# urw7rs/diffusion-models-made-easy

Measured on AMD Instinct MI355X. Metric: denoising steps/sec + training images/sec, DDPM UNet CIFAR10 32×32 @1/2/4/8 GPU, higher is better.
Workload: dtype bf16; 1 GPU; DDPM T=1000 sampling, CIFAR10 32x32, default UNet (32,416,643 params, random init), batch 128 per GPU, t.shape=(1,); global_batch=128, parallelism=dp1 (independent chains per GPU, no data-path collective)

## Files before the change

### diffusion-models-made-easy_amd/_lib.py

```python

from __future__ import annotations

import ctypes as C
import os
import subprocess
import threading

_HERE = os.path.dirname(os.path.abspath(__file__))
LIB_PATH = os.environ.get("DMME_LIB_PATH") or os.path.join(_HERE, "libdmme_hip.so")
CSRC = os.path.join(_HERE, "csrc")

F16R32 = 4
F32, BF16, BF16X3, F16 = 0, 1, 2, 3
CHAIN_DDPM, CHAIN_DDIM, CHAIN_IDDPM, CHAIN_DDPM_GUIDED, CHAIN_DDIM_GUIDED, CHAIN_GDDIM = 0, 1, 2, 3, 4, 5
CHAIN_DDPM_CFG, CHAIN_GDDIM_CFG = 6, 7
CHAIN_DPMPP, CHAIN_DPMPP_CFG = 8, 9
CHAIN_REPAINT = 10
PRED_EPS, PRED_X0, PRED_V = 0, 1, 2
PREDICTIONS = {"eps": PRED_EPS, "x0": PRED_X0, "v": PRED_V}
THRESHOLD_NONE, THRESHOLD_STATIC, THRESHOLD_DYNAMIC = 0, 1, 2
THRESHOLDS = {"none": THRESHOLD_NONE, "static": THRESHOLD_STATIC, "dynamic": THRESHOLD_DYNAMIC}
ARCH_DDPM, ARCH_IDDPM, ARCH_CLASSIFIER, ARCH_DDPM_COND = 0, 1, 2, 3
DTYPES = {"fp32": F32, "float32": F32, "32": F32, "bf16": BF16, "bfloat16": BF16, "16": BF16, "bf16-mixed": BF16, "16-mixed": BF16,
          "bf16x3": BF16X3, "fp16": F16, "float16": F16, "half": F16, "fp16r32": F16R32}
# ... 37 lines not shown
    cmd = ["make", "-C", CSRC, "-j", str(min(8, os.cpu_count() or 1))]
    res = subprocess.run(cmd, stdout=subprocess.PIPE, stderr=subprocess.STDOUT, text=True)
    if verbose or res.returncode != 0:
        print(res.stdout)
    if res.returncode != 0:
        raise DmmeError("building libdmme_hip.so failed")
    return LIB_PATH


_vp, _i, _i64, _f, _u64 = C.c_void_p, C.c_int, C.c_int64, C.c_float, C.c_uint64

PROTOTYPES = {
    "dmme_last_error": (C.c_char_p, []),
    "dmme_version": (_i, []),
    "dmme_device_count": (_i, []),
    "dmme_unet_plan_create": (_i, [C.POINTER(UNetCfg), _i, _i, _i, _i, _i, C.POINTER(_vp)]),
    "dmme_unet_plan_destroy": (None, [_vp]),
    "dmme_unet_plan_num_params": (_i, [_vp]),
    "dmme_unet_plan_param_info": (_i, [_vp, _i, C.c_char_p, _i, C.POINTER(_i), C.POINTER(_i64), C.POINTER(_i64), C.POINTER(_i)]),
    "dmme_unet_plan_ref_numel": (_i64, [_vp]),
    "dmme_unet_plan_packed_bytes": (_i64, [_vp]),
    "dmme_unet_plan_workspace_bytes": (_i64, [_vp]),
    "dmme_unet_plan_dropmask_numel": (_i64, [_vp]),
    "dmme_unet_plan_out_channels": (_i, [_vp]),
    "dmme_unet_plan_num_launches": (_i, [_vp]),
    "dmme_unet_plan_num_launches_nograd": (_i, [_vp]),
    "dmme_unet_plan_num_folded": (_i, [_vp]),
    "dmme_unet_pack_params": (_i, [_vp, _vp, _vp, _vp]),
    "dmme_unet_pack_folded": (_i, [_vp, _vp, _vp]),
    "dmme_unet_forward": (_i, [_vp, _vp, _vp, _vp, _i, _vp, _vp, _vp, _vp]),
    "dmme_unet_forward_nograd": (_i, [_vp, _vp, _vp, _vp, _i, _vp, _vp, _vp, _vp]),
    "dmme_unet_forward_cond": (_i, [_vp, _vp, _vp, _vp, _i, _vp, _vp, _vp, _vp, _i, _vp, _vp]),
    "dmme_unet_backward_cond": (_i, [_vp, _vp, _vp, _vp, _vp, _i, _vp, _vp, _vp, _vp, _vp, _vp, _vp, _vp, _vp, _vp]),
    "dmme_unet_backward_input_cond": (_i, [_vp, _vp, _vp, _vp, _vp, _i, _vp, _vp, _vp, _vp, _vp, _vp, _vp]),
    "dmme_label_dropout": (_i, [_vp, _i, _i, _f, _u64, _u64, _vp, _vp, _vp]),
    "dmme_cfg_step": (_i, [_i, _vp, _vp, _vp, _f, _f, _f, _f, _i, _i, _i64, _vp]),
    "dmme_chain_update_cfg": (_i, [_i, _vp, _vp, _vp, _vp, _vp, _vp, _i, _i64, _vp]),
    "dmme_cfg_chain_step": (_i, [_vp, _vp, _vp, _vp, _vp, _vp, _vp, _i, _vp, _vp, _vp, _vp]),
    "dmme_dpmpp_step": (_i, [_vp, _vp, _vp, C.POINTER(_f), _i, _i, _i64, _i, _vp]),
    "dmme_chain_update_dpmpp": (_i, [_vp, _vp, _vp, _vp, _vp, _vp, _i, _i64, _i, _vp]),
    "dmme_dpmpp_chain_step": (_i, [_vp, _vp, _vp, _vp, _vp, _vp, _vp, _vp, _vp, _vp]),
    "dmme_cfg_dpmpp_step": (_i, [_vp, _vp, _vp, C.POINTER(_f), _i, _i, _i64, _vp]),
    "dmme_chain_update_cfg_dpmpp": (_i, [_vp, _vp, _vp, _vp, _vp, _vp, _i, _i64, _vp]),
    "dmme_cfg_dpmpp_chain_step": (_i, [_vp, _vp, _vp, _vp, _vp, _vp, _vp, _vp, _vp, _vp, _vp, _vp]),
    "dmme_repaint_step": (_i, [_vp, _vp, _vp, _vp, _vp, C.POINTER(_f), _i, _i64, _i, _vp]),
    "dmme_chain_update_repaint": (_i, [_vp, _vp, _vp, _vp, _vp, _vp, _vp, _vp, _i, _i64, _i, _vp]),
    "dmme_repaint_chain_step": (_i, [_vp, _vp, _vp, _vp, _vp, _vp, _vp, _vp, _vp, _vp, _vp]),
    "dmme_unet_plan_num_ops": (_i, [_vp]),
    "dmme_unet_plan_level_info": (_i, [_vp, C.c_char_p, _i]),
    "dmme_unet_plan_check": (_i, [_vp]),
    "dmme_debug_level_stamps": (_i, [_vp, _i, _i]),
    "dmme_unet_plan_op_info": (_i, [_vp, _i, C.c_char_p, _i, C.POINTER(C.c_double), C.POINTER(C.c_double)]),
    "dmme_unet_forward_profiled": (_i, [_vp, _vp, _vp, _vp, _i, _vp, _vp, _vp, _vp, _vp]),
    "dmme_unet_plan_packed_bwd_bytes": (_i64, [_vp]),
    "dmme_unet_plan_bwd_workspace_bytes": (_i64, [_vp]),
    "dmme_unet_pack_params_bwd": (_i, [_vp, _vp, _vp, _vp]),
    "dmme_unet_backward": (_i, [_vp, _vp, _vp, _vp, _vp, _i, _vp, _vp, _vp, _vp, _vp, _vp, _vp]),
    "dmme_unet_backward_buckets": (_i, [_vp, _vp, _vp, _vp, _vp, _i, _vp, _vp, _vp, _vp, _vp, _vp, _vp, BUCKET_FN, _vp]),
    "dmme_unet_backward_input": (_i, [_vp, _vp, _vp, _vp, _vp, _i, _vp, _vp, _vp, _vp, _vp, _vp]),
    "dmme_unet_plan_grad_buckets": (_i, [_vp, C.POINTER(_i64), C.POINTER(_i64), C.POINTER(_i), _i]),
    "dmme_unet_plan_bwd_summary": (_i, [_vp, C.c_char_p, _i]),
    "dmme_grad_norm": (_i, [_vp, _i64, _vp, _vp, _vp]),
    "dmme_adam_step": (_i, [_vp, _vp, _vp, _vp, _vp, _i64, _f, _f, _f, _f, _i, _vp, _f, _f, _f, _vp]),
    "dmme_amp_init": (_i, [_vp, _f, _vp]),
    "dmme_amp_scale": (_i, [_vp, _i64, _vp, _vp]),
    "dmme_adam_step_amp": (_i, [_vp, _vp, _vp, _vp, _vp, _i64, _f, _f, _f, _f, _vp, _f, _f, _f, _vp, _f, _f, _i, _vp]),
    "dmme_grad_pack_bf16": (_i, [_vp, _i64, _vp, _i64, _vp]),
    "dmme_shard_reduce_bf16": (_i, [_vp, _i, _i64, _f, _vp, _vp]),
    "dmme_grad_unpack_bf16": (_i, [_vp, _i64, _vp, _vp]),
    "dmme_unet_debug_read": (_i, [_vp, _vp, C.c_char_p, _vp, _i64, C.POINTER(_i64), _vp]),
    "dmme_unet_debug_read_grad": (_i, [_vp, _vp, C.c_char_p, _vp, _i64, C.POINTER(_i64), _vp]),
    "dmme_unet_debug_read_norm_stats": (_i, [_vp, _vp, C.c_char_p, _vp, _i64, C.POINTER(_i64), _vp]),
    "dmme_dropout_masks": (_i, [_vp, _u64, _u64, _vp, _vp]),
    "dmme_randn": (_i, [_vp, _i64, _u64, _u64, _vp]),
    "dmme_q_sample": (_i, [_vp, _vp, _vp, _vp, _vp, _i, _i64, _vp, _vp, _vp]),
    "dmme_ddpm_step": (_i, [_vp, _vp, _vp, _f, _f, _f, _i, _i64, _vp]),
    "dmme_ddim_step": (_i, [_vp, _vp, _f, _f, _i64, _vp]),
    "dmme_gddim_step": (_i, [_vp, _vp, _vp, _f, _f, _f, _i64, _vp]),
    "dmme_slerp": (_i, [_vp, _vp, _vp, _i, _i, _i64, _vp, _vp]),
    "dmme_chain_set": (_i, [_vp, _i64, _vp, _u64, _u64, _vp]),
    "dmme_chain_update": (_i, [_i, _vp, _vp, _vp, _vp, _vp, _i, _i64, _vp]),
    "dmme_chain_step": (_i, [_vp, _vp, _vp, _vp, _vp, _i, _vp, _vp, _vp, _vp]),
    "dmme_chain_update_gddim": (_i, [_vp, _vp, _vp, _vp, _vp, _vp, _i, _i64, _vp]),
    "dmme_log_softmax_grad": (_i, [_vp, _vp, _i, _i, _i, _f, _vp, _vp, _vp, _vp]),
    "dmme_chain_update_guided": (_i, [_i, _vp, _vp, _vp, _vp, _vp, _vp, _vp, _i, _i64, _vp]),
    "dmme_guided_chain_step": (_i, [_vp, _vp, _vp, _vp, _vp, _vp, _vp, _vp, _vp, _vp, _vp, _vp, _vp, _vp, _vp, _i, _vp, _vp, _vp, _vp]),
    "dmme_mse_loss": (_i, [_vp, _vp, _i64, _vp, _vp, _f, _vp, _vp]),
    "dmme_pred_to_eps": (_i, [_i, _vp, _vp, _vp, _i, _vp, _i, _i, _i64, _vp]),
    "dmme_unet_plan_set_prediction": (_i, [_vp, _i, _vp, _i]),
    "dmme_x0_threshold": (_i, [_i, _vp, _vp, _vp, _i, _vp, _i, _i, _i64, _i, _i, _f, _i, _f, _vp, _vp]),
    "dmme_x0_threshold_scratch_bytes": (_i64, [_i, _i64]),
    "dmme_x0_threshold_lds_capacity": (_i, []),
    "dmme_unet_plan_set_threshold": (_i, [_vp, _i, _vp, _i, _i, _f, _vp]),
    "dmme_q_sample_pred": (_i, [_i, _vp, _vp, _vp, _vp, _vp, _i, _i64, _vp, _vp, _vp]),
    "dmme_mse_loss_rows": (_i, [_vp, _vp, _vp, _vp, _i, _i64, _vp, _vp, _f, _vp, _vp]),
    "dmme_image_batch": (_i, [_vp, _i64, _vp, _vp, _i, _i, _i, _i, _vp, _vp]),
    "dmme_grid_tile": (_i, [_vp, _i, _i, _i, _i, _i, _i, _i, _i, _i, _i, _i, _vp, _vp]),
    "dmme_iddpm_step": (_i, [_vp, _vp, _vp, _f, _f, _f, _f, _i, _i, _i64, _vp]),
    "dmme_iddpm_loss": (_i, [_vp, _vp, _vp, _vp, _vp, _vp, _i, _i64, _f, _f, _vp, _vp, _f, _vp, _vp]),
    "dmme_iddpm_loss_rows": (_i, [_vp, _vp, _vp, _vp, _vp, _vp, _i, _vp, _i, _i64, _f, _f, _vp, _vp, _vp, _f, _vp, _vp, _vp]),
    "dmme_iddpm_prior_rows": (_i, [_vp, _i, _i64, _f, _vp, _vp]),
    "dmme_tsampler_draw": (_i, [_vp, _vp, _i, _i, _f, _u64, _u64, _i, _vp, _vp, _vp, _vp]),
    "dmme_tsampler_update": (_i, [_vp, _vp, _i, _i, _vp, _vp, _i, _vp, _vp]),
    "dmme_conv2d": (_i, [C.POINTER(ConvDesc), _vp, _vp, _vp, _vp, _vp, _vp, _vp, _vp, _vp, _vp, _i, _vp, _vp]),
    "dmme_conv2d_res": (_i, [C.POINTER(ConvDesc), _vp, _vp, _vp, _vp, _vp, _vp, _vp, _vp, _vp, _i, _i, _vp, _vp, _vp, _vp]),
    "dmme_groupnorm_scale_shift": (_i, [_i, _vp, _vp, _i, _i, _i, _i, _i, _vp, _vp, _f, _vp, _vp, _vp, _i, _vp]),
    "dmme_attention": (_i, [_i, _vp, _i, _i, _i, _vp, _i, _vp]),
    "dmme_attention_proj": (_i, [_i, _vp, _i, _i, _i, _vp, _vp, _vp, _vp, _vp, _vp, _i, _vp]),
    "dmme_attention_fold": (_i, [_i, _i, _vp, _vp, _vp, _vp, _vp, _vp, _vp, _vp, _vp]),
    "dmme_attention_block": (_i, [_i, _vp, _i, _i, _i, _vp, _i, _i, _i, _vp, _vp, _f, _vp, _vp, _vp, _vp, _vp, _vp, _vp, _vp, _vp, _i, _vp]),
    "dmme_attention_heads": (_i, [_i, _vp, _i, _i, _i, _i, _vp, _i, _vp]),
    "dmme_nchw_to_nhwc": (_i, [_i, _vp, _i, _i, _i, _vp, _vp]),
    "dmme_nhwc_to_nchw": (_i, [_i, _vp, _i, _i, _i, _vp, _vp]),
    "dmme_pack_weight": (_i, [_i, _vp, _i, _i, _i, _vp, _vp]),
    "dmme_event_create": (_i, [C.POINTER(_vp)]),
    "dmme_event_record": (_i, [_vp, _vp]),
    "dmme_event_elapsed_ms": (_i, [_vp, _vp, C.POINTER(_f)]),
    "dmme_event_destroy": (_i, [_vp]),
    "dmme_debug_set_stamps": (_i, [_vp]),
    "dmme_debug_mfma_valu": (_i, [_i, _i, _i, _vp, _vp]),
    "dmme_debug_issue_probe": (_i, [_i, _i, _i, _i, _i, _vp, _vp, _vp]),
    "dmme_debug_l2_stream": (_i, [_vp, _i64, _i, _i, _i, _i, _vp, _vp]),
}


def lib():
    global _lib
    if _lib is not None:
        return _lib
    with _lock:
        if _lib is not None:
            return _lib
        if not os.path.exists(LIB_PATH):
            raise DmmeError(
                f"{LIB_PATH} is missing: the HIP extension is not built. Run `python -c 'import __graft_entry__ as g; g.build()'` "
                "(or `make -C diffusion-models-made-easy_amd/csrc`). There is no CPU fallback for the product path."
            )
        h = C.CDLL(LIB_PATH)
        for name, (res, args) in PROTOTYPES.items():
            fn = getattr(h, name)
            fn.restype = res
            fn.argtypes = args
        _lib = h
    return _lib


def check(rc: int, what: str = ""):
    if rc != 0:
        msg = lib().dmme_last_error().decode("utf-8", "replace")
        if rc == -2:
            raise NotImplementedError(f"{what}: {msg}")
        if rc == -1:
            raise ValueError(f"{what}: {msg}")
        raise DmmeError(f"{what} failed (status {rc}): {msg}")


def require_gpu():
    if lib().dmme_device_count() <= 0:
        raise DmmeError("libdmme_hip.so loaded but no HIP device is visible; the denoiser path only runs on an MI355X")


def dtype_code(precision) -> int:
    key = str(precision).lower()
    if key not in DTYPES:
        raise ValueError(f"unknown precision {precision!r}; use 'fp32', 'bf16', 'fp16' / 'fp16r32' (inference) or 'bf16x3'")
    return DTYPES[key]
# ... 25 lines not shown
```

### diffusion-models-made-easy_amd/csrc/common.h

```cpp
#pragma once

#include <hip/hip_runtime.h>
#include <stdint.h>

#include "dmme_hip.h"

namespace dmme {

void set_error(const char* fmt, ...) __attribute__((format(printf, 1, 2)));

int debug_route(const char* key, int dflt = 0);

#define DMME_CHECK_HIP(expr)                                                                          \
    do {                                                                                              \
        hipError_t e_ = (expr);                                                                       \
        if (e_ != hipSuccess) {                                                                       \
            ::dmme::set_error("%s failed: %s (%s:%d)", #expr, hipGetErrorString(e_), __FILE__, __LINE__); \
            return DMME_ERR_HIP;                                                                      \
        }                                                                                             \
    } while (0)

#define DMME_REQUIRE(cond, code, ...)        \
    do {                                     \
        if (!(cond)) {                       \
// ... 257 lines not shown
int conv_gn_direct_query(int dtype, const ConvArgs& a, const int* cg, int n);
int launch_gn_finalize_parts(const float* part1, int tiles1, int cnt1, int C1, const float* part2, int tiles2, int cnt2, int C2, int N, int groups,
                             const float* gamma, const float* beta, float eps, float* scale, float* shift, float* mean_rstd, const float* t_shift,
                             const float* t_scale, int t_ld, int nt, hipStream_t s);

int launch_gn_generic(int dtype, const void* src1, const void* src2, int N, int HW, int C1, int C2, int groups,
                      const float* gamma, const float* beta, float eps, float* scale, float* shift, float* mean_rstd,
                      hipStream_t s);
bool gn_fast_supported(int dtype, int N, int HW, int C1, int C2, int groups);
size_t gn_fast_scratch_floats(int N, int HW, int C, int groups);
int launch_gn_fast(int dtype, const void* src1, const void* src2, int N, int HW, int C1, int C2, int groups,
                   const float* gamma, const float* beta, float eps, float* scale, float* shift, float* mean_rstd,
                   float* partial, hipStream_t s, void* act = nullptr, int act_silu = 0, const float* dmask = nullptr);
bool gn_small_act_supported(int dtype, int HW, int C1, int C2, int groups);

int launch_attn_generic(int dtype, const void* qkv, int N, int S, int C, void* out, hipStream_t s);
int launch_attn_heads(int dtype, const void* qkv, int N, int S, int C, int heads, void* out, hipStream_t s);
int launch_attn_heads_bwd(int dtype, const void* qkv, const void* dO, int N, int S, int C, int heads, float* P, float* dS, void* dqkv, hipStream_t s);
int launch_gn_modulate(float* scale, float* shift, const float* t_shift, const float* t_scale, int ld, int nt, int N, int C, hipStream_t s);
bool attn_x3_supported(int N, int S, int C, int heads);
int launch_attn_x3(const void* qkv, int N, int S, int C, int heads, void* out, hipStream_t s);
bool attn_mfma_supported(int dtype, int N, int S, int C);
bool attn_full_takes(int S, int D);
int launch_attn_mfma(int dtype, const void* qkv, int N, int S, int C, void* out, float* lse, hipStream_t s);
bool attn_proj_fusable(int dtype, int N, int S, int C, int gn_cg, int gn_tiles);
int launch_attn_proj(int dtype, const void* qkv, int N, int S, int C, void* ctx, float* lse, const void* w, const float* bias, const void* res, void* dst,
                     float* gn_part, int gn_tiles, int gn_cg, hipStream_t s, long long* stamps = nullptr);
struct AttnFoldJob {
    int64_t wq, bq, wp, bp;
    int64_t M, c, wpv, bias2;
    int32_t C, pad;
};
bool attn_fold_shape_ok(int dtype, int N, int S, int C, int gn_cg, int gn_tiles);
int launch_attn_fold(int dtype, const void* x, int N, int S, int C, const GnIn* gni, const float* scale, const float* shift, const void* M, const float* c,
                     const void* wpv, const float* bias2, const void* res, void* dst, float* gn_part, int gn_tiles, int gn_cg, hipStream_t s,
                     long long* stamps = nullptr);
int launch_attn_fold_weights(int dtype, const AttnFoldJob* jobs_dev, int n_jobs, int maxC, void* packed, hipStream_t s, const AttnFoldJob* one = nullptr);
bool attn_heads_mfma_supported(int dtype, int N, int S, int C, int heads);
int launch_attn_heads_mfma(int dtype, const void* qkv, int N, int S, int C, int heads, void* out, float* lse, hipStream_t s);
int launch_attn_heads_bwd_mfma(int dtype, const void* qkv, const void* O, const void* dO, const float* lse, int N, int S, int C, int heads, void* P,
                               void* dS, void* dqkv, hipStream_t s);
bool attn_bwd_mfma_supported(int dtype, int N, int S, int C);
int launch_attn_bwd_mfma(int dtype, const void* qkv, const void* O, const void* dO, const float* lse, int N, int S, int C, void* P, void* dS,
                         void* dqkv, hipStream_t s);

constexpr unsigned kFwdMarkKeep = 0x4B454550u, kFwdMarkNograd = 0x4E4F4752u;
constexpr unsigned kErrNogradBackward = 0x80000000u;
int launch_time_sinusoid(const int64_t* t, int nt, const float* freqs, int half, float* out, hipStream_t s, unsigned* mark = nullptr,
                         unsigned mark_val = 0);
int launch_linear_wave(int dtype, const float* in, int nt, int K, const void* W, const float* bias, int Nout,
                       int out_silu, float* out, hipStream_t s);
int launch_label_cond(const float* z2, int nt, const float* E, const int64_t* labels, int B, int K, int emb, float* temb, float* zsave, int* status,
                      hipStream_t s);
int launch_label_grad(const float* dz2, const int64_t* labels, int B, int K, int emb, float* dE, hipStream_t s);

int launch_nchw_to_nhwc(int dtype, const float* src, int N, int C, int HW, void* dst, hipStream_t s, const unsigned* mark = nullptr,
                        unsigned* err = nullptr);
int launch_nhwc_to_nchw(int dtype, const void* src, int N, int C, int HW, float* dst, hipStream_t s);
int launch_pack_weight(int dtype, const float* src, int Cout, int Cin, int taps, void* dst, hipStream_t s);
int launch_cast_f32_to_16(int dtype, const float* src, int64_t numel, void* dst, hipStream_t s);

struct PackItem {
    int64_t src_off;
    int64_t dst_off;
    int32_t cout, cin, taps;
    int32_t row0, rows;
    int32_t ci0, nci;
    int32_t as_f32;
};
int launch_pack_table(int dtype, const PackItem* items_dev, int n_items, const float* ref_flat, void* packed,
                      hipStream_t s);

int launch_randn(float* out, int64_t numel, uint64_t seed, uint64_t offset, hipStream_t s);
int launch_dropmask(float* out, int64_t numel, float p, uint64_t seed, uint64_t offset, hipStream_t s);
int launch_q_sample(const float* x0, const float* z, const float* sqrt_abar, const float* sqrt_1m_abar,
                    const int64_t* t, int B, int64_t chw, float* x_t, float* target, hipStream_t s);
int launch_pred_to_eps(int pred, float* model_out, const float* x, const float* ab, int T, const int64_t* t, int t_len, int B, int64_t chw,
                       hipStream_t s);
int launch_x0_threshold(int mode, float* out, const float* x, const float* table, int T, const int64_t* t, int t_len, int B, int64_t chw, int planes,
                        int halves, float sg, const float* sg_coef, int sg_row, int sg_col, const int64_t* sg_state, int k, float frac, void* scratch,
                        hipStream_t s);
int slerp_parts(int64_t chw);
int launch_slerp(const float* xa, const float* xb, const float* w, int n, int B, int64_t chw, float* out, float* scratch, hipStream_t s);
int launch_chain_set(void* state, int64_t i, const int64_t* t_table, uint64_t seed, uint64_t offset, hipStream_t s);

constexpr bool kind_known(int k) { return k >= DMME_CHAIN_DDPM && k <= DMME_CHAIN_REPAINT; }
constexpr bool kind_cfg(int k) { return k == DMME_CHAIN_DDPM_CFG || k == DMME_CHAIN_GDDIM_CFG || k == DMME_CHAIN_DPMPP_CFG; }
__device__ __forceinline__ float cfg_mix(float e_c, float e_u, float s) { return __fadd_rn(e_u, __fmul_rn(s, __fsub_rn(e_c, e_u))); }
constexpr int kind_base(int k) {
    return k == DMME_CHAIN_DDPM_CFG ? DMME_CHAIN_DDPM : k == DMME_CHAIN_GDDIM_CFG ? DMME_CHAIN_GDDIM : k == DMME_CHAIN_DPMPP_CFG ? DMME_CHAIN_DPMPP : k;
}
constexpr bool kind_hist(int k) { return kind_base(k) == DMME_CHAIN_DPMPP; }
constexpr bool kind_paint(int k) { return k == DMME_CHAIN_REPAINT; }
constexpr int kind_row(int k) { return kind_hist(k) || kind_paint(k) ? 8 : 4; }
constexpr int kind_scol(int k) { return kind_hist(k) ? 6 : 3; }
constexpr bool kind_grad(int k) { return k == DMME_CHAIN_DDPM_GUIDED || k == DMME_CHAIN_DDIM_GUIDED; }
constexpr int kind_planes(int k) { return k == DMME_CHAIN_IDDPM ? 2 : k == DMME_CHAIN_DPMPP || kind_paint(k) ? 0 : 1; }
enum { NOISE_NEVER, NOISE_NOT_LAST, NOISE_C2, NOISE_ROW };
constexpr int kind_noise(int k) {
    return kind_paint(k) ? NOISE_ROW : kind_hist(k) || k == DMME_CHAIN_DDIM || k == DMME_CHAIN_DDIM_GUIDED ? NOISE_NEVER : kind_base(k) == DMME_CHAIN_GDDIM ? NOISE_C2 : NOISE_NOT_LAST;
}
constexpr int kind_adds_noise(int k, float c2, int not_last) { return kind_noise(k) == NOISE_C2 ? c2 != 0.0f : kind_noise(k) == NOISE_NOT_LAST ? not_last : 0; }
constexpr int paint_streams_used(float c2, float ks, float r1) { return (c2 != 0.0f ? 1 : 0) | (ks != 0.0f ? 2 : 0) | (r1 != 0.0f ? 4 : 0); }
constexpr int kind_streams(int k) { return kind_paint(k) ? 3 : 1; }
constexpr bool kind_draws(int k, int flag, int s) { return kind_paint(k) ? ((flag >> s) & 1) != 0 : kind_noise(k) != NOISE_NEVER && flag != 0; }
constexpr bool kind_zin(int k) { return k == DMME_CHAIN_DDPM_GUIDED || kind_base(k) == DMME_CHAIN_GDDIM || k == DMME_CHAIN_DDPM_CFG || kind_paint(k); }
constexpr bool kind_ragged(int k) { return k == DMME_CHAIN_DDPM || k == DMME_CHAIN_DDIM || k == DMME_CHAIN_GDDIM || k == DMME_CHAIN_IDDPM; }

struct SamplerOperands {
    float* x;
    const float* out;
    const float* grad;
    const float* zin;
    float* hist;
    const float* known;
    const float* mask;
    int64_t chw, numel, n4;
    int planes;
};
int launch_sampler_eager(const char* what, int kind, const SamplerOperands& o, const float* row, int flag, hipStream_t s);
int launch_sampler_chain(const char* what, int kind, const SamplerOperands& o, const float* coef, const int64_t* t_table, void* state, hipStream_t s);
int launch_label_dropout(const int64_t* labels, int B, int K, float p, uint64_t seed, uint64_t offset, int64_t* out, int* status, hipStream_t s);
int launch_cls_head_fwd(int dtype, const void* top, int B, int HW, int C, int G, const float* gamma, const float* beta, const float* W,
                        const float* bias, int K, float* logits, hipStream_t s);
int launch_cls_head_bwd(int dtype, const void* top, int B, int HW, int C, int G, const float* gamma, const float* beta, const float* W, int K,
                        const float* dlog, void* dtop, float* pooled, float* rows, hipStream_t s);
int launch_cls_head_wgrad(const float* dlog, const float* pooled, const float* rows, int B, int K, int C, float* dW, float* db, float* dgamma,
                          float* dbeta, hipStream_t s);
int launch_log_softmax_grad(const float* logits, const int64_t* y, int B, int K, int mode, float scale, float* loss, float* dlog, int* status,
                            hipStream_t s);
int launch_image_batch(const uint8_t* data, const int64_t* idx, const uint8_t* flip, int B, int C, int H, int W, float* out, hipStream_t s);
int launch_grid_tile(const float* x, int B, int C, int H, int W, int cell0, int cell_stride, int xmaps, int ymaps, int pad, int out_kind, int raw,
                     void* canvas, hipStream_t s);
int launch_iddpm_loss(const float* out, const float* x_t, const float* x_0, const float* target, const int64_t* t, const float* coef, int B,
                      int64_t chw, float w_simple, float w_vlb, float* loss, float* d_out, float gscale, float* scratch, hipStream_t s);
int launch_iddpm_loss_rows(const float* out, const float* x_t, const float* x_0, const float* target, const int64_t* t, const float* coef, int T,
                           const float* weight, int B, int64_t chw, float w_simple, float w_vlb, float* loss, float* rows, float* d_out,
                           float gscale, int* status, float* scratch, hipStream_t s);
int launch_iddpm_prior_rows(const float* x_0, int B, int64_t chw, float alpha_bar_T, float* prior, hipStream_t s);
int launch_tsampler_draw(const float* hist, const int* count, int T, int H, float uniform_prob, uint64_t seed, uint64_t offset, int B, int64_t* t,
                         float* weight, float* p, hipStream_t s);
int launch_tsampler_update(float* hist, int* count, int T, int H, const int64_t* t, const float* L, int B, int* status, hipStream_t s);
int launch_mse(const float* eps, const float* target, int64_t numel, float* loss, float* d_eps, float gscale,
               float* scratch, hipStream_t s);

int launch_wgrad_generic(int dtype, const ConvArgs& a, const void* dY, float* dW, hipStream_t s);
bool wgrad_small_supported(int dtype, const ConvArgs& a);
int launch_wgrad_small(int dtype, const ConvArgs& a, const void* dY, float* dW, hipStream_t s);
bool wgrad_mfma_supported(int dtype, const ConvArgs& a);
int launch_wgrad_mfma(int dtype, const ConvArgs& a, const void* dY, float* dWp, hipStream_t s);
struct PackItem;

struct WgLayer {
    int64_t src1_off, src2_off;
    int64_t scale_off, shift_off;
    int64_t dmask_off;
    int64_t dy_off;
    int64_t dw_off;
    int64_t act_off;
    int act_bws;
    int N, Hin, Win, C1, C2, up, Hout, Wout, Cout, pro_silu;
    int shTW, shTH;
    int ks_off[4], half_off;
    int ks_row[4], half_row;
    ConvTile g;
};
struct WgJob {
    int layer, cot, cit, tile0, ntiles;
};
bool wgrad_group_layer(int dtype, const ConvArgs& a, WgLayer& L, int* co_tile, int* ci_tile);
int launch_wgrad_group(int dtype, int taps, const WgLayer* layers_dev, const WgJob* jobs_dev, int njobs, const void* ws, const void* bws,
                       const float* drop_masks, float* wimage, hipStream_t s, int dma = 0, const void* zero_page = nullptr);
int launch_wgrad_unpack(const PackItem* items_dev, int n_items, const float* image, float* grad_flat, hipStream_t s);
int launch_colsum(int dtype, const void* dY, int N, int HW, int C, float* rowsum, float* dbias, float* dtproj, int ld, int nt,
                  hipStream_t s);
struct GnMod {
    const float* t_scale = nullptr;
    const float* beta = nullptr;
    float* d_shift = nullptr;
    float* d_scale = nullptr;
    int ld = 0, nt = 0;
#if defined(__HIPCC__)
    __device__ __forceinline__ float mul(int n, int c) const { return t_scale ? 1.0f + t_scale[(int64_t)(nt == 1 ? 0 : n) * ld + c] : 1.0f; }
    __device__ __forceinline__ void emit(int n, int c, float A, float B, float gamma_c) const {
        if (!t_scale) return;
        const float ds = fmaf(gamma_c, B, beta[c] * A);
        if (nt == 1) {
            atomicAdd(&d_shift[c], A);
            atomicAdd(&d_scale[c], ds);
        } else {
            d_shift[(int64_t)n * ld + c] = A;
            d_scale[(int64_t)n * ld + c] = ds;
        }
    }
#endif
};
int launch_gn_bwd_generic(int dtype, const void* dv, const void* x1, const void* x2, int N, int HW, int C1, int C2, int groups,
                          const float* gamma, const float* mean_rstd, const float* scale, const float* shift, const float* dmask,
                          int pro_silu, void* dx1, void* dx2, int acc1, int acc2, float* dgamma, float* dbeta, GnMod mod, hipStream_t s);
bool colsum_fast_supported(int dtype, int HW, int C);
struct BiasJob {
    int64_t rowsum_off;
    int64_t dbias_off;
    int C, cblock, tcol;
// ... 56 lines not shown
```

### diffusion-models-made-easy_amd/csrc/kernels_sampler.hip

```cpp
#include "common.h"

#include <type_traits>

namespace dmme {

struct Philox {
    uint32_t c[4];
    uint32_t k[2];
};
__device__ __forceinline__ void philox_round(uint32_t (&c)[4], uint32_t k0, uint32_t k1) {
    const uint64_t p0 = (uint64_t)0xD2511F53u * c[0];
    const uint64_t p1 = (uint64_t)0xCD9E8D57u * c[2];
    const uint32_t n0 = (uint32_t)(p1 >> 32) ^ c[1] ^ k0;
    const uint32_t n1 = (uint32_t)p1;
    const uint32_t n2 = (uint32_t)(p0 >> 32) ^ c[3] ^ k1;
    const uint32_t n3 = (uint32_t)p0;
    c[0] = n0;
    c[1] = n1;
    c[2] = n2;
    c[3] = n3;
}
__device__ __forceinline__ void philox4x32_10(uint64_t seed, uint64_t ctr, uint32_t (&out)[4]) {
    uint32_t c[4] = {(uint32_t)ctr, (uint32_t)(ctr >> 32), 0u, 0u};
    uint32_t k0 = (uint32_t)seed, k1 = (uint32_t)(seed >> 32);
// ... 61 lines not shown
    if (numel <= 0) return DMME_OK;
    hipLaunchKernelGGL(dropmask_kernel, dim3(grid_for((numel + 3) / 4)), dim3(256), 0, s, out, numel, p, seed, offset);
    DMME_CHECK_LAUNCH();
    return DMME_OK;
}

__global__ void __launch_bounds__(256) q_sample_kernel(const float* __restrict__ x0, const float* __restrict__ z,
                                                       const float* __restrict__ sqrt_abar,
                                                       const float* __restrict__ sqrt_1m_abar,
                                                       const int64_t* __restrict__ t, int64_t chw, int64_t total,
                                                       float* __restrict__ x_t, float* __restrict__ target) {
    for (int64_t i = blockIdx.x * (int64_t)blockDim.x + threadIdx.x; i < total; i += (int64_t)gridDim.x * blockDim.x) {
        const int64_t tn = t[i / chw];
        const float sa = sqrt_abar[tn], sd = sqrt_1m_abar[tn];
        const float mean = sa * x0[i];
        const float xt = mean + sd * z[i];
        x_t[i] = xt;
        if (target) target[i] = (xt - mean) / sd;
    }
}
int launch_q_sample(const float* x0, const float* z, const float* sqrt_abar, const float* sqrt_1m_abar,
                    const int64_t* t, int B, int64_t chw, float* x_t, float* target, hipStream_t s) {
    const int64_t total = (int64_t)B * chw;
    if (total <= 0) return DMME_OK;
    hipLaunchKernelGGL(q_sample_kernel, dim3(grid_for(total)), dim3(256), 0, s, x0, z, sqrt_abar, sqrt_1m_abar, t, chw, total,
                       x_t, target);
    DMME_CHECK_LAUNCH();
    return DMME_OK;
}

__device__ __forceinline__ float ddpm_mean(float x, float e, float c0, float c1) { return __fmul_rn(c0, __fsub_rn(x, __fmul_rn(c1, e))); }
__device__ __forceinline__ float ddim_collapse(float x, float e, float c0, float c1) {
    return __fmul_rn(c1, __fdiv_rn(__fsub_rn(x, __fmul_rn(c0, e)), c1));
}
__device__ __forceinline__ float iddpm_std(float v, float log_beta, float log_beta_tilde) {
    return sqrtf(expf(__fadd_rn(__fmul_rn(v, log_beta), __fmul_rn(__fsub_rn(1.0f, v), log_beta_tilde))));
}
template <int KIND>
__device__ __forceinline__ float sampler_update(float x, float e, float v, float g, float z, float c0, float c1, float c2, float c3, int add_noise) {
    if (KIND == DMME_CHAIN_DDIM) return ddim_collapse(x, e, c0, c1);
    if (KIND == DMME_CHAIN_DDIM_GUIDED) return ddim_collapse(x, __fsub_rn(e, __fmul_rn(c2, g)), c0, c1);
    float m;
    if (KIND == DMME_CHAIN_GDDIM) {
        m = __fadd_rn(__fmul_rn(c0, x), __fmul_rn(c1, e));
    } else {
        m = ddpm_mean(x, e, c0, c1);
        if (KIND == DMME_CHAIN_DDPM_GUIDED) m = __fadd_rn(m, __fmul_rn(c3, g));
    }
    return add_noise ? __fadd_rn(m, __fmul_rn(KIND == DMME_CHAIN_IDDPM ? iddpm_std(v, c2, c3) : c2, z)) : m;
}
struct DpmppRow {
    float q0, q1, k0, k1, w, clip, s;
};
__device__ __forceinline__ float dpmpp_update(float x, float e, float prev, const DpmppRow& r, bool valid, float& x0) {
    x0 = __fadd_rn(__fmul_rn(r.q0, x), __fmul_rn(r.q1, e));
    if (r.clip != 0.0f) x0 = fminf(fmaxf(x0, -1.0f), 1.0f);
    const float d = valid ? __fadd_rn(x0, __fmul_rn(r.w, __fsub_rn(x0, prev))) : x0;
    return __fadd_rn(__fmul_rn(r.k0, x), __fmul_rn(r.k1, d));
}
struct PaintRow {
    float c0, c1, c2, ka, ks, r0, r1;
};
__device__ __forceinline__ float paint_update(float x, float e, float x0, float m, float z0, float z1, float z2, const PaintRow& r, int used) {
    float u = ddpm_mean(x, e, r.c0, r.c1);
    if (used & 1) u = __fadd_rn(u, __fmul_rn(r.c2, z0));
    float k = __fmul_rn(r.ka, x0);
    if (used & 2) k = __fadd_rn(k, __fmul_rn(r.ks, z1));
    const float y = __fadd_rn(__fmul_rn(m, k), __fmul_rn(__fsub_rn(1.0f, m), u));
    return used & 4 ? __fadd_rn(__fmul_rn(r.r0, y), __fmul_rn(r.r1, z2)) : y;
}
__device__ __forceinline__ float4 load4(const float* p) { return *reinterpret_cast<const float4*>(p); }

struct ChainState {
    long long i;
    long long t;
    unsigned long long offset;
    unsigned long long seed;
    unsigned int ticket, pad;
    unsigned long long history_valid;
    unsigned long long reserved[2];
};
static_assert(sizeof(ChainState) == 64, "ChainState is eight 64-bit words (dmme_hip.h: dmme_chain_*)");

__global__ void chain_set_kernel(ChainState* st, long long i, const long long* __restrict__ t_table, unsigned long long seed, unsigned long long offset) {
    st->i = i;
    st->t = t_table[i];
    st->offset = offset;
    st->seed = seed;
    st->ticket = 0u;
    st->pad = 0u;
    st->history_valid = 0ull;
}
int launch_chain_set(void* state, int64_t i, const int64_t* t_table, uint64_t seed, uint64_t offset, hipStream_t s) {
    hipLaunchKernelGGL(chain_set_kernel, dim3(1), dim3(1), 0, s, (ChainState*)state, (long long)i, (const long long*)t_table, (unsigned long long)seed,
                       (unsigned long long)offset);
    DMME_CHECK_LAUNCH();
    return DMME_OK;
}

__device__ __forceinline__ void chain_advance(ChainState* st, const long long* __restrict__ t_table, long long i, unsigned long long offset_inc,
                                              bool raise_history) {
    if (threadIdx.x != 0) return;
    const unsigned tk = atomicAdd(&st->ticket, 1u);
    if (tk != gridDim.x - 1) return;
    const long long ni = i > 0 ? i - 1 : 0;
    st->i = ni;
    st->t = t_table[ni];
    if (offset_inc) st->offset += offset_inc;
    if (raise_history) st->history_valid = 1ull;
    atomicExch(&st->ticket, 0u);
}

struct Row {
    float c[8];
};

template <bool DRAWS>
__device__ __forceinline__ void noise4(bool add_noise, const float* zin, int64_t b, uint64_t seed, uint64_t ctr, float (&z)[4]) {
    z[0] = z[1] = z[2] = z[3] = 0.f;
    if (!add_noise) return;
    if (!DRAWS || zin) {
        const float4 zv = load4(zin + b);
        z[0] = zv.x; z[1] = zv.y; z[2] = zv.z; z[3] = zv.w;
    } else {
        normal4(seed, ctr, z);
    }
}

template <int KIND, bool DRAWS>
__device__ __forceinline__ void step_noise(const SamplerOperands& o, int flag, const float* zin, int64_t q, uint64_t seed, uint64_t off,
                                           float (&z)[4 * kind_streams(KIND)]) {
    if constexpr (kind_streams(KIND) == 1) {
        noise4<DRAWS>(kind_draws(KIND, flag, 0), zin, q * 4, seed, off + (uint64_t)q, z);
    } else {
#pragma unroll
        for (int s = 0; s < kind_streams(KIND); ++s)
            noise4<DRAWS>(kind_draws(KIND, flag, s), zin ? zin + s * o.numel : nullptr, q * 4, seed, off + (uint64_t)s * (uint64_t)o.n4 + (uint64_t)q,
                          *reinterpret_cast<float(*)[4]>(z + 4 * s));
    }
}

template <int KIND>
__device__ __forceinline__ void update_quad(const SamplerOperands& o, int64_t q, const Row& r, int flag, const float (&z)[4 * kind_streams(KIND)]) {
    const int64_t b = q * 4;
    const int planes = kind_planes(KIND) ? kind_planes(KIND) : o.planes;
    const int64_t eo = planes == 2 ? b + (b / o.chw) * o.chw : b;
    float4 xv = load4(o.x + b), ev = load4(o.out + eo), av = make_float4(0.f, 0.f, 0.f, 0.f);
    float *xs = reinterpret_cast<float*>(&xv), *es = reinterpret_cast<float*>(&ev), *as = reinterpret_cast<float*>(&av);
    if constexpr (kind_cfg(KIND)) {
        const float4 uv = load4(o.out + o.n4 * 4 + b);
        const float* us = reinterpret_cast<const float*>(&uv);
#pragma unroll
        for (int j = 0; j < 4; ++j) es[j] = cfg_mix(es[j], us[j], r.c[kind_scol(KIND)]);
    }
    if constexpr (kind_hist(KIND)) {
        const DpmppRow d = {r.c[0], r.c[1], r.c[2], r.c[3], r.c[4], r.c[5], r.c[6]};
        if (flag) av = load4(o.hist + b);
#pragma unroll
        for (int j = 0; j < 4; ++j) xs[j] = dpmpp_update(xs[j], es[j], as[j], d, flag != 0, as[j]);
        *reinterpret_cast<float4*>(o.hist + b) = av;
    } else if constexpr (kind_paint(KIND)) {
        const PaintRow p = {r.c[0], r.c[1], r.c[2], r.c[3], r.c[4], r.c[5], r.c[6]};
        const float4 mv = load4(o.mask + b);
        av = load4(o.known + b);
        const float* ms = reinterpret_cast<const float*>(&mv);
#pragma unroll
        for (int j = 0; j < 4; ++j) xs[j] = paint_update(xs[j], es[j], as[j], ms[j], z[j], z[4 + j], z[8 + j], p, flag);
    } else {
        constexpr bool LEARNED = KIND == DMME_CHAIN_IDDPM;
        if (LEARNED && flag) av = load4(o.out + eo + o.chw);
        if (kind_grad(KIND)) av = load4(o.grad + b);
#pragma unroll
        for (int j = 0; j < 4; ++j)
            xs[j] = sampler_update<kind_base(KIND)>(xs[j], es[j], LEARNED ? as[j] : 0.f, kind_grad(KIND) ? as[j] : 0.f, z[j], r.c[0], r.c[1], r.c[2],
                                                    kind_cfg(KIND) ? 0.f : r.c[3], flag);
    }
    *reinterpret_cast<float4*>(o.x + b) = xv;
    if (kind_cfg(KIND)) *reinterpret_cast<float4*>(o.x + o.n4 * 4 + b) = xv;
}

template <int KIND>
__global__ void __launch_bounds__(256) eager_kernel(SamplerOperands o, Row r, int flag) {
    const bool quads_fit = KIND != DMME_CHAIN_IDDPM || o.chw % 4 == 0;
    for (int64_t q = blockIdx.x * (int64_t)blockDim.x + threadIdx.x; q < o.n4; q += (int64_t)gridDim.x * blockDim.x) {
        const int64_t b = q * 4;
        if (!kind_ragged(KIND) || (b + 3 < o.numel && quads_fit)) {
            float z[4 * kind_streams(KIND)];
            step_noise<KIND, false>(o, flag, o.zin, q, 0, 0, z);
            update_quad<KIND>(o, q, r, flag, z);
        } else if constexpr (kind_ragged(KIND)) {
            for (int64_t i = b; i < b + 4 && i < o.numel; ++i) {
                const int64_t eo = KIND == DMME_CHAIN_IDDPM ? i + (i / o.chw) * o.chw : i;
                o.x[i] = sampler_update<KIND>(o.x[i], o.out[eo], KIND == DMME_CHAIN_IDDPM && flag ? o.out[eo + o.chw] : 0.f, 0.f, flag ? o.zin[i] : 0.f,
                                              r.c[0], r.c[1], r.c[2], r.c[3], flag);
            }
        }
    }
}

template <int KIND>
__global__ void __launch_bounds__(256) __attribute__((amdgpu_waves_per_eu(8))) chain_kernel(SamplerOperands o, const float* __restrict__ coef, const long long* __restrict__ t_table, ChainState* st) {
    const long long i = st->i, t = st->t;
    const unsigned long long off = st->offset, seed = st->seed;
    Row r;
#pragma unroll
    for (int j = 0; j < kind_row(KIND); ++j) r.c[j] = coef[kind_row(KIND) * i + j];
    const int flag = kind_hist(KIND) ? st->history_valid != 0ull : kind_paint(KIND) ? paint_streams_used(r.c[2], r.c[4], r.c[6]) : kind_adds_noise(KIND, r.c[2], t != 1);
    for (int64_t q = blockIdx.x * (int64_t)blockDim.x + threadIdx.x; q < o.n4; q += (int64_t)gridDim.x * blockDim.x) {
        float z[4 * kind_streams(KIND)];
        step_noise<KIND, true>(o, flag, kind_zin(KIND) ? o.zin : nullptr, q, seed, off, z);
        update_quad<KIND>(o, q, r, flag, z);
    }
    __syncthreads();
    chain_advance(st, t_table, i, kind_hist(KIND) ? 0ull : (unsigned long long)o.n4 * kind_streams(KIND), kind_hist(KIND));
}

template <int K = 0, class F>
static int dispatch_kind(int kind, F&& f) {
    if constexpr (K > DMME_CHAIN_REPAINT) {
        set_error("unknown sampler kind %d", kind);
        return DMME_ERR_INVALID;
    } else {
        return kind == K ? f(std::integral_constant<int, K>{}) : dispatch_kind<K + 1>(kind, f);
    }
}
static int check_operands(const char* what, int kind, const SamplerOperands& o, bool eager) {
    DMME_REQUIRE(kind_known(kind), DMME_ERR_INVALID, "%s: unknown sampler kind %d", what, kind);
    DMME_REQUIRE(o.x && o.out && (o.hist || !kind_hist(kind)) && ((o.known && o.mask) || !kind_paint(kind)) && o.numel > 0 && o.chw > 0, DMME_ERR_INVALID,
                 "%s: bad argument", what);
    DMME_REQUIRE(kind_grad(kind) == (o.grad != nullptr), DMME_ERR_INVALID, "%s: the guided kinds (3, 4) and only they take a gradient", what);
    DMME_REQUIRE(kind_planes(kind) || o.planes == 1 || o.planes == 2, DMME_ERR_INVALID, "%s: a network output of %d planes per image (1: eps, 2: eps and v)",
                 what, o.planes);
    DMME_REQUIRE((eager && kind_ragged(kind)) || o.chw % 4 == 0, DMME_ERR_UNSUPPORTED, "%s: image size %lld is not a multiple of 4", what, (long long)o.chw);
    return DMME_OK;
}
int launch_sampler_eager(const char* what, int kind, const SamplerOperands& o, const float* row, int flag, hipStream_t s) {
    if (kind_ragged(kind) && o.numel <= 0) return DMME_OK;
    if (int rc = check_operands(what, kind, o, true)) return rc;
    DMME_REQUIRE(row, DMME_ERR_INVALID, "%s: null argument", what);
    Row r = {};
    for (int j = 0; j < kind_row(kind); ++j) r.c[j] = row[j];
    if (!kind_hist(kind)) flag = kind_paint(kind) ? paint_streams_used(r.c[2], r.c[4], r.c[6]) : kind_adds_noise(kind, r.c[2], flag);
    DMME_REQUIRE(o.zin || kind_hist(kind) || !flag, DMME_ERR_INVALID, "%s: a step that adds noise needs z", what);
    return dispatch_kind(kind, [&](auto k) -> int {
        constexpr int K = decltype(k)::value;
        if constexpr (kind_grad(K)) {
            set_error("%s: the guided kinds have no eager form", what);
            return DMME_ERR_INVALID;
        } else {
            hipLaunchKernelGGL(eager_kernel<K>, dim3(grid_for(o.n4)), dim3(256), 0, s, o, r, flag);
            DMME_CHECK_LAUNCH();
            return DMME_OK;
        }
    });
}
int launch_sampler_chain(const char* what, int kind, const SamplerOperands& o, const float* coef, const int64_t* t_table, void* state, hipStream_t s) {
    if (int rc = check_operands(what, kind, o, false)) return rc;
    DMME_REQUIRE(coef && t_table && state, DMME_ERR_INVALID, "%s: null argument", what);
    return dispatch_kind(kind, [&](auto k) -> int {
        hipLaunchKernelGGL(chain_kernel<decltype(k)::value>, dim3(grid_for(o.n4)), dim3(256), 0, s, o, coef, (const long long*)t_table, (ChainState*)state);
        DMME_CHECK_LAUNCH();
        return DMME_OK;
    });
}

__global__ void __launch_bounds__(256) mse_partial_kernel(const float* __restrict__ eps, const float* __restrict__ target,
                                                          int64_t numel, float* __restrict__ d_eps, float gscale,
                                                          float* __restrict__ partial) {
    __shared__ float red[16];
    float acc = 0.f;
    for (int64_t i = blockIdx.x * (int64_t)blockDim.x + threadIdx.x; i < numel; i += (int64_t)gridDim.x * blockDim.x) {
        const float d = target[i] - eps[i];
        acc += d * d;
        if (d_eps) d_eps[i] = (-2.0f * d) * gscale;
    }
    const float tot = block_sum(acc, red);
    if (threadIdx.x == 0) partial[blockIdx.x] = tot;
}
__global__ void __launch_bounds__(256) mse_final_kernel(const float* partial, int n, float inv_numel, float* loss) {
    __shared__ float red[16];
    float acc = 0.f;
    for (int i = threadIdx.x; i < n; i += blockDim.x) acc += partial[i];
    const float tot = block_sum(acc, red);
    if (threadIdx.x == 0) loss[0] = tot * inv_numel;
}
int launch_mse(const float* eps, const float* target, int64_t numel, float* loss, float* d_eps, float gscale,
               float* scratch, hipStream_t s) {
    DMME_REQUIRE(numel > 0, DMME_ERR_INVALID, "mse: numel must be positive");
    unsigned g = grid_for(numel);
    if (g > 1024) g = 1024;
    hipLaunchKernelGGL(mse_partial_kernel, dim3(g), dim3(256), 0, s, eps, target, numel, d_eps,
                       gscale / (float)numel, scratch);
    DMME_CHECK_LAUNCH();
    hipLaunchKernelGGL(mse_final_kernel, dim3(1), dim3(256), 0, s, scratch, (int)g, 1.0f / (float)numel, loss);
    DMME_CHECK_LAUNCH();
    return DMME_OK;
}

__device__ __forceinline__ void iddpm_loss_elem(const float* __restrict__ c, bool t_is_one, float e, float v, float xt, float x0, float tgt,
                                                float& d, float& vlb, float& dv) {
    d = tgt - e;
    const float mean = c[0] * (xt - c[1] * e);
    const float sd = iddpm_std(v, c[2], c[3]);
    const float hl = 0.5f * (c[2] - c[3]);
    if (t_is_one) {
        const float ap = (x0 + 1.0f / 255.0f - mean) / sd, am = (x0 - 1.0f / 255.0f - mean) / sd;
        const bool up = x0 < 1.0f, lo = x0 > -1.0f;
        const float Fp = up ? 0.5f * (1.0f + erff(ap * 0.70710678118654752f)) : 1.0f;
        const float Fm = lo ? 0.5f * (1.0f + erff(am * 0.70710678118654752f)) : 0.0f;
        const float prob = Fp - Fm;
        vlb = -logf(fmaxf(prob, 1e-12f));
        const float pp = up ? 0.3989422804014327f * expf(-0.5f * ap * ap) * ap : 0.f;
        const float pm = lo ? 0.3989422804014327f * expf(-0.5f * am * am) * am : 0.f;
        dv = prob >= 1e-12f ? hl * (pp - pm) / prob : 0.f;
    } else {
        const float qm = c[4] * x0 + c[5] * xt;
        const float q = c[6] / sd, ratio = q * q;
        const float u = (qm - mean) / sd, t1 = u * u;
        vlb = 0.5f * (ratio + t1 - 1.0f - logf(ratio));
        dv = hl * (1.0f - ratio - t1);
    }
}
__global__ void __launch_bounds__(256) iddpm_loss_kernel(const float* __restrict__ out, const float* __restrict__ x_t, const float* __restrict__ x_0,
                                                         const float* __restrict__ target, const int64_t* __restrict__ t,
                                                         const float* __restrict__ coef, int64_t chw, int64_t total, float w_simple, float w_vlb,
                                                         float gscale, float* __restrict__ d_out, float* __restrict__ partial) {
    __shared__ float red[16];
    float acc_s = 0.f, acc_v = 0.f;
    for (int64_t i = blockIdx.x * (int64_t)blockDim.x + threadIdx.x; i < total; i += (int64_t)gridDim.x * blockDim.x) {
        const int64_t b = i / chw, r = i - b * chw;
        const int64_t tt = t[b];
        float d, vlb, dv;
        iddpm_loss_elem(coef + tt * 8, tt == 1, out[b * 2 * chw + r], out[b * 2 * chw + chw + r], x_t[i], x_0[i], target[i], d, vlb, dv);
        acc_s += d * d;
        acc_v += vlb;
        if (d_out) {
            d_out[b * 2 * chw + r] = (-2.0f * d) * (w_simple * gscale);
            d_out[b * 2 * chw + chw + r] = dv * (w_vlb * gscale);
        }
    }
    const float ts = block_sum(acc_s, red);
    __syncthreads();
    const float tv = block_sum(acc_v, red);
// ... 471 lines not shown
```

### diffusion-models-made-easy_amd/csrc/plan.h

```cpp
#pragma once
#include <stdarg.h>
#include <stdlib.h>
#include <stdio.h>
#include <string.h>

#include <algorithm>
#include <memory>
#include <string>
#include <unordered_map>
#include <vector>

#include "common.h"
#include "lvl.h"

namespace dmme {

static inline int64_t align_up(int64_t v, int64_t a) { return (v + a - 1) / a * a; }

template <typename T>
class DevTable {
    T* p_ = nullptr;

public:
    DevTable() = default;
// ... 115 lines not shown
    DevTable<unsigned> sync_dev;
    double flops = 0, bytes = 0;
};

}

using namespace dmme;

struct dmme_plan {
    dmme_unet_cfg cfg;
    int B, H, W, dtype, device;
    int x3 = 0;
    int mix = 0;
    int out_channels = 0;
    int head_src = -1, p_hgw = -1, p_hgb = -1, p_hw = -1, p_hb = -1;
    int64_t bws_hpool = 0, bws_hrows = 0;
    int cond = 0, p_lemb = -1, label_op = -1;
    std::vector<Param> params;
    std::vector<Tensor> tensors;
    std::vector<Op> ops;
    std::unordered_map<std::string, int> named;
    int64_t ref_numel = 0, packed_bytes = 0, ws_bytes = 0, dropmask_numel = 0;
    int64_t ws_tsin = 0, ws_th1 = 0, ws_temb = 0, ws_tproj = 0, ws_gnpart = 0;
    int64_t ws_mark = 0;
    int64_t ws_tz1 = -1, ws_tz2 = -1;
    int64_t ws_splitk = 0, splitk_floats = 0;
    int tproj_cols = 0;
    int64_t tproj_w_off = 0, tproj_b_off = 0;
    int freqs_param = -1;
    DevTable<PackItem> items_dev;
    int n_items = 0;
    int n_launches = 0;
    struct TBlock { int tw, tb, col, cout; };
    std::vector<TBlock> tblocks;
    int p_l1w = -1, p_l1b = -1, p_l2w = -1, p_l2b = -1;
    int64_t packed_bwd_bytes = 0, bws_bytes = 0;
    std::vector<int64_t> gt_off;
    int64_t bws_zero = 0, bws_zero_bytes = 0, bws_wimage = 0, bws_gnS = 0, bws_zpage = 0;
    DevTable<PackItem> items_unpack_dev;
    int n_items_unpack = 0;
    int64_t bws_sink = 0, sink_half = 0;
    int64_t bws_tmp = 0, bws_dy = 0, bws_rowsum = 0, bws_dtproj = 0, bws_dtemb = 0, bws_dh1 = 0, bws_z = 0, bws_wT = 0, bws_attP = 0,
            bws_attdS = 0;
    DevTable<PackItem> items_bwd_dev;
    int n_items_bwd = 0;
    struct WgGroup {
        int taps = 0;
        std::vector<WgLayer> layers;
        std::vector<WgJob> jobs;
        DevTable<WgLayer> layers_dev;
        DevTable<WgJob> jobs_dev;
        int dma = 0;
        int stride = 1;
    } wg[3];
    struct GradBucket {
        int op_lo = 0, op_hi = 0;
        WgGroup wg[3];
        int col0 = 0, col1 = 0, bias0 = 0, bias1 = 0;
        std::vector<std::pair<int, int>> unpack, tcols;
        std::vector<std::pair<int64_t, int64_t>> ranges;
    };
    std::vector<GradBucket> gb;
    std::vector<int64_t> tp_tiles;
    DevTable<int64_t> tp_tiles_dev;
    int tp_n64 = 0;
    std::vector<BiasJob> bias_jobs;
    DevTable<BiasJob> bias_jobs_dev;
    std::vector<ColJob> col_jobs;
    DevTable<ColJob> col_jobs_dev;
    std::vector<LvlRun> lvl_runs;
    int lvl_max_wg = LVL_MAX_WG;
    PinnedWord err_host;
    mutable const void* nograd_ws = nullptr;
    std::vector<AttnFoldJob> fold_jobs;
    DevTable<AttnFoldJob> fold_jobs_dev;
    int fold_maxC = 0, n_launches_nograd = 0;
    mutable const void* fold_packed = nullptr;
    int pred = DMME_PRED_EPS, pred_T = 0;
    const float* pred_ab = nullptr;
    int thr_mode = DMME_THRESHOLD_NONE, thr_T = 0, thr_k = 0;
    float thr_frac = 0.f;
    const float* thr_table = nullptr;
    void* thr_scratch = nullptr;
};

namespace dmme {

constexpr int kR32TwoPassDefault = 0;
static inline int conv_dt(const dmme_plan* P, const Op& o) { return o.route_f32 ? DMME_F32 : P->dtype; }
static inline int wg_index(const Op& o) { return o.taps == 1 ? 1 : o.stride == 2 ? 2 : 0; }

void fill_conv(const dmme_plan* P, const Op& o, const char* packed, const float* x, float* y, char* ws, const float* drop_masks, int nt, ConvArgs& a,
               bool fwd = false);
bool gn_from_parts(const dmme_plan* P, const Op& o);
void assign_levels(dmme_plan* P);
void assign_rseg(dmme_plan* P);
int run_level(const dmme_plan* P, const LvlRun& R, const char* pk, char* ws, int nt, const float* drop_masks, hipStream_t s, bool keep_ctx = true);
void assign_lvl_nograd(dmme_plan* P);
void assign_attn_fold(dmme_plan* P);
int lvl_check(const dmme_plan* P, const char* where, hipStream_t stream = nullptr, bool have_stream = false);
void build_unpack_items(const dmme_plan* P, std::vector<PackItem>& items);
void plan_backward(dmme_plan* P);

}
```

### diffusion-models-made-easy_amd/csrc/plan.hip

```cpp
#include "plan.h"

#include <functional>
#include <map>
#include <mutex>

namespace dmme {

static thread_local char g_err[512] = "";
void set_error(const char* fmt, ...) {
    va_list ap;
    va_start(ap, fmt);
    vsnprintf(g_err, sizeof(g_err), fmt, ap);
    va_end(ap);
}

int debug_route(const char* key, int dflt) {
    const char* e = getenv("DMME_DEBUG_ROUTE");
    if (!e || !*e) return dflt;
    const size_t kl = strlen(key);
    for (const char* p = e; *p;) {
        const char* end = strchr(p, ',');
        const size_t len = end ? (size_t)(end - p) : strlen(p);
        if (len >= kl && !strncmp(p, key, kl) && (len == kl || p[kl] == '=')) return len == kl ? 1 : atoi(p + kl + 1);
        if (!end) break;
// ... 470 lines not shown
            const int64_t v = (int64_t)B * to.H * to.W * (cin > to.C ? cin : to.C);
            if (v > mx) mx = v;
        }
        P->splitk_floats = 4 * mx;
        P->ws_splitk = ws_alloc(P->splitk_floats * 4 + 16);
    }
    P->ws_bytes = ws;
    P->n_launches = (int)ops.size();

    return DMME_OK;
}

static void push_pack_items(const Param& p, int64_t dst_off, int as_f32, bool wide_co, std::vector<PackItem>& items) {
    const int LIMIT = 8192;
    int nco, nci;
    if (as_f32 == 1) {
        nci = p.cin;
        nco = LIMIT / (p.cin * p.taps);
        if (nco < 1) nco = 1;
    } else if (wide_co) {
        nco = p.cout < 64 ? p.cout : 64;
        nci = LIMIT / (nco * p.taps);
        if (nci > p.cin) nci = p.cin;
        if (nci >= 4) nci &= ~3;
        if (nci < 1) nci = 1;
    } else {
        nci = p.cin;
        if (nci * p.taps > LIMIT) nci = LIMIT / p.taps;
        nco = LIMIT / (nci * p.taps);
        if (nco < 1) nco = 1;
    }
    if (as_f32 != 1 && nco > 256) nco = 256;
    for (int r0 = 0; r0 < p.cout; r0 += nco)
        for (int c0 = 0; c0 < p.cin; c0 += nci) {
            PackItem it;
            it.src_off = p.ref_off;
            it.dst_off = dst_off;
            it.cout = p.cout;
            it.cin = p.cin;
            it.taps = p.taps;
            it.row0 = r0;
            it.rows = p.cout - r0 < nco ? p.cout - r0 : nco;
            it.ci0 = c0;
            it.nci = p.cin - c0 < nci ? p.cin - c0 : nci;
            it.as_f32 = as_f32;
            items.push_back(it);
        }
}

void build_pack_items(const dmme_plan* P, std::vector<PackItem>& items) {
    for (const Param& p : P->params) push_pack_items(p, p.packed_off, p.pack_code >= 0 ? p.pack_code : p.as_f32 ? 1 : 0, false, items);
}

void build_pack_items_bwd(const dmme_plan* P, std::vector<PackItem>& items) {
    for (const Param& p : P->params)
        if (p.packed_bwd_off >= 0) push_pack_items(p, p.packed_bwd_off, 2, true, items);
}

void build_unpack_items(const dmme_plan* P, std::vector<PackItem>& items) {
    const int64_t CHUNK = 16384;
    for (const Param& p : P->params) {
        if (p.wp_off < 0) continue;
        const int64_t row = (int64_t)p.cin * p.taps;
        int64_t rows_per = CHUNK / row;
        if (rows_per < 1) rows_per = 1;
        for (int64_t r0 = 0; r0 < p.cout; r0 += rows_per) {
            PackItem it;
            it.src_off = p.ref_off;
            it.dst_off = p.wp_off;
            it.cout = p.cout;
            it.cin = p.cin;
            it.taps = p.taps;
            it.row0 = (int32_t)r0;
            it.rows = (int32_t)((p.cout - r0) < rows_per ? (p.cout - r0) : rows_per);
            it.ci0 = 0;
            it.nci = p.cin;
            it.as_f32 = 0;
            items.push_back(it);
        }
    }
}

void fill_conv(const dmme_plan* P, const Op& o, const char* packed, const float* x, float* y, char* ws,
               const float* drop_masks, int nt, ConvArgs& a, bool fwd) {
    const int64_t es = (int64_t)dtype_size(P->dtype);
    (void)es;
    a.x3 = P->x3 || o.route_f32;
    a.f16 = P->dtype == DMME_F16 && !o.route_f32;
    a.mix = o.mix;
    a.mix2 = o.mix2;
    a.N = P->B;
    if (o.src1 == -2) {
        a.src1 = x;
        a.in_nchw = 1;
        a.C1 = P->cfg.in_channels;
        a.Hin = P->H;
        a.Win = P->W;
    } else {
        const Tensor& t = P->tensors[o.src1];
        a.src1 = ws + t.off;
        a.C1 = t.C;
        a.Hin = t.H;
        a.Win = t.W;
    }
    if (o.src2 >= 0) {
        a.src2 = ws + P->tensors[o.src2].off;
        a.C2 = P->tensors[o.src2].C;
    }
    const Param& w = P->params[o.w];
    a.w = packed + w.packed_off;
    a.bias = (const float*)(packed + P->params[o.b].packed_off);
    a.Cout = w.cout;
    a.taps = o.taps;
    a.stride = o.stride;
    a.up = o.up;
    const int Hv = o.up ? 2 * a.Hin : a.Hin, Wv = o.up ? 2 * a.Win : a.Win;
    a.Hout = Hv / o.stride;
    a.Wout = Wv / o.stride;
    if (o.gn >= 0) {
        a.scale = (const float*)(ws + P->ops[o.gn].gn_scale);
        a.shift = (const float*)(ws + P->ops[o.gn].gn_shift);
        const Op& g = P->ops[o.gn];
        if (fwd && g.gn_in_consumer) {
            const Tensor& t1 = P->tensors[g.gn_src1];
            const Tensor* t2 = g.gn_src2 >= 0 ? &P->tensors[g.gn_src2] : nullptr;
            a.has_gni = 1;
            a.gni.p1 = (const float*)(ws + t1.stats_off);
            a.gni.t1 = t1.stats_tiles;
            a.gni.cnt1 = t1.stats_cnt;
            a.gni.C1 = t1.C;
            a.gni.p2 = t2 ? (const float*)(ws + t2->stats_off) : nullptr;
            a.gni.t2 = t2 ? t2->stats_tiles : 0;
            a.gni.cnt2 = t2 ? t2->stats_cnt : 0;
            a.gni.C2 = t2 ? t2->C : 0;
            a.gni.groups = P->cfg.num_groups;
            a.gni.gamma = (const float*)(packed + P->params[g.gn_gamma].packed_off);
            a.gni.beta = (const float*)(packed + P->params[g.gn_beta].packed_off);
            a.gni.eps = 1e-5f;
            a.gni.mean_rstd = (float*)(ws + g.gn_mr);
            if (g.gn_mod_col >= 0) {
                a.gni.t_shift = (const float*)(ws + P->ws_tproj) + g.gn_mod_col;
                a.gni.t_scale = a.gni.t_shift + g.gn_mod_C;
                a.gni.t_ld = P->tproj_cols;
                a.gni.nt = nt;
            }
        }
    }
    a.pro_silu = o.pro_silu;
    a.out_silu = o.out_silu;
    if (o.dmask_off >= 0 && drop_masks) a.dmask = drop_masks + o.dmask_off;
    if (fwd && o.use_act) {
        a.src1 = ws + P->ops[o.gn].gn_act;
        a.C1 = a.C1 + a.C2;
        a.src2 = nullptr;
        a.C2 = 0;
        a.scale = a.shift = a.dmask = nullptr;
        a.pro_silu = 0;
    }
    if (o.tproj_col >= 0) {
        a.tproj = (const float*)(ws + P->ws_tproj) + o.tproj_col;
        a.tproj_ld = P->tproj_cols;
        a.nt = nt;
    }
    if (fwd && o.rseg >= 0) {
        const Op& rc = P->ops[o.rseg];
        const Tensor& r1 = P->tensors[rc.src1];
        a.r_src1 = ws + r1.off;
        a.r_C1 = r1.C;
        if (rc.src2 >= 0) {
            a.r_src2 = ws + P->tensors[rc.src2].off;
            a.r_C2 = P->tensors[rc.src2].C;
        }
        a.r_w = packed + P->params[rc.w].packed_off;
        a.r_bias = (const float*)(packed + P->params[rc.b].packed_off);
    } else if (o.res1 >= 0) {
        a.res1 = ws + P->tensors[o.res1].off;
        a.R1 = P->tensors[o.res1].C;
        if (o.res2 >= 0) a.res2 = ws + P->tensors[o.res2].off;
    }
    if (P->splitk_floats > 0 && ws) {
        a.splitk = (float*)(ws + P->ws_splitk);
        a.splitk_cap = P->splitk_floats;
    }
    if (fwd && o.gd_n > 0) {
        a.n_gno = o.gd_n;
        a.gn_eps = 1e-5f;
        a.gn_cg = P->tensors[o.dst].C / P->cfg.num_groups;
        for (int k = 0; k < o.gd_n; ++k) {
            const Op& g = P->ops[o.gd_gn[k]];
            GnOut& G = a.gno[k];
            G.gamma = (const float*)(packed + P->params[g.gn_gamma].packed_off);
            G.beta = (const float*)(packed + P->params[g.gn_beta].packed_off);
            G.scale = (float*)(ws + g.gn_scale);
            G.shift = (float*)(ws + g.gn_shift);
            G.mean_rstd = (float*)(ws + g.gn_mr);
            G.C = P->tensors[g.gn_src1].C + (g.gn_src2 >= 0 ? P->tensors[g.gn_src2].C : 0);
            G.cg = G.C / P->cfg.num_groups;
            G.c_off = o.gd_coff[k];
            if (k == o.gd_act) {
                const Op& cv = P->ops[g.gn_consumer];
                a.act = ws + g.gn_act;
                a.act_k = k;
                a.act_silu = cv.pro_silu;
                a.act_dmask = (cv.dmask_off >= 0 && drop_masks) ? drop_masks + cv.dmask_off : nullptr;
            }
        }
    }
    a.gn_raw_moments = P->mix ? 1 : 0;
    if (o.dst == -2) {
        a.dst = y;
        a.out_nchw = 1;
    } else {
        const Tensor& td = P->tensors[o.dst];
        a.dst = ws + td.off;
        if (td.stats_off >= 0) {
            a.gn_part = (float*)(ws + td.stats_off);
            a.gn_cg = td.C / P->cfg.num_groups;
            a.gn_tiles = td.stats_tiles;
        }
    }
}

bool gn_from_parts(const dmme_plan* P, const Op& o) {
    if (o.gn_force_small) return false;
    const Tensor& t1 = P->tensors[o.gn_src1];
    if (t1.stats_off < 0) return false;
    const int G = P->cfg.num_groups;
    int C = t1.C;
    if (o.gn_src2 >= 0) {
        const Tensor& t2 = P->tensors[o.gn_src2];
        if (t2.stats_off < 0) return false;
        C += t2.C;
        const int cg = C / G;
        if (t1.C % cg || cg % (t1.C / G) || cg % (t2.C / G)) return false;
    }
    return true;
}

void assign_stats(dmme_plan* P) {
    std::vector<char> wanted(P->tensors.size(), 0);
    for (const Op& o : P->ops)
        if (o.kind == OP_GN && o.lvl < 0) {
            wanted[o.gn_src1] = 1;
// ... 178 lines not shown
            rc.fused_away = 1;
        }
    next:;
    }
}

void assign_attn_proj(dmme_plan* P) {
    if (P->x3) return;
    for (int ai = 0; ai + 1 < (int)P->ops.size(); ++ai) {
        Op& at = P->ops[ai];
        if (at.kind != OP_ATTN || at.lvl >= 0 || at.at_heads != 1) continue;
        Op& pr = P->ops[ai + 1];
        if (pr.kind != OP_CONV || pr.src1 != at.at_out || pr.src2 >= 0 || pr.taps != 1 || pr.lvl >= 0 || pr.gn >= 0 || pr.pro_silu || pr.out_silu || pr.dmask_off >= 0 ||
            pr.tproj_col >= 0 || pr.res1 < 0 || pr.res2 >= 0 || pr.up || pr.stride != 1 || pr.gd_n > 0 || pr.mix || pr.route_f32 || pr.dst < 0 || pr.fused_away || pr.rseg >= 0)
            continue;
        const Tensor &q = P->tensors[at.at_qkv], &td = P->tensors[pr.dst];
        if (q.f32 || td.f32 || P->tensors[pr.res1].f32 || P->tensors[at.at_out].f32) continue;
        const int S = q.H * q.W, C = q.C / 3;
        if (td.C != C || P->tensors[pr.res1].C != C) continue;
        const bool stats = td.stats_off >= 0;
        if (!attn_proj_fusable(P->dtype, P->B, S, C, stats ? td.C / P->cfg.num_groups : 0, stats ? td.stats_tiles : 0)) continue;
        at.at_proj = ai + 1;
        pr.fused_away = 2;
    }
}

void assign_attn_fold(dmme_plan* P) {
    if (getenv("DMME_NO_ATTN_FOLD") || debug_route("no_attn_fold") || !is16(P->dtype) || P->x3 || P->mix) return;
    int64_t cur = P->packed_bytes;
    const int64_t es = (int64_t)dtype_size(P->dtype);
    for (int ai = 1; ai < (int)P->ops.size(); ++ai) {
        Op& at = P->ops[ai];
        if (at.kind != OP_ATTN || at.at_proj < 0 || at.at_heads != 1 || at.lvl >= 0) continue;
        Op& qc = P->ops[ai - 1];
        const Op& pr = P->ops[at.at_proj];
        if (qc.kind != OP_CONV || qc.dst != at.at_qkv || qc.taps != 1 || qc.src1 < 0 || qc.src2 >= 0 || qc.gn < 0 || qc.pro_silu || qc.out_silu || qc.dmask_off >= 0 ||
            qc.tproj_col >= 0 || qc.res1 >= 0 || qc.res2 >= 0 || qc.up || qc.stride != 1 || qc.gd_n > 0 || qc.mix || qc.route_f32 || qc.fused_away || qc.rseg >= 0 ||
            qc.use_act || qc.lvl >= 0 || pr.res1 != qc.src1)
            continue;
        const Op& gn = P->ops[qc.gn];
        const Tensor& tx = P->tensors[qc.src1];
        const int C = tx.C, groups = P->cfg.num_groups;
        if (gn.kind != OP_GN || gn.gn_src1 != qc.src1 || gn.gn_src2 >= 0 || gn.gn_mod_col >= 0 || gn.gn_act >= 0 || tx.f32 ||
            (gn.gn_in_consumer && (tx.stats_off < 0 || tx.stats_tiles > 32)) || P->tensors[at.at_qkv].C != 3 * C || P->params[qc.w].pack_code >= 0 || P->params[pr.w].pack_code >= 0)
            continue;
        bool only_here = true;
        for (int oi = 0; oi < (int)P->ops.size() && only_here; ++oi) {
            const Op& o = P->ops[oi];
            if (oi == ai) continue;
            if (o.kind == OP_CONV && (o.src1 == at.at_qkv || o.src2 == at.at_qkv || o.res1 == at.at_qkv || o.res2 == at.at_qkv)) only_here = false;
            if (o.kind == OP_GN && (o.gn_src1 == at.at_qkv || o.gn_src2 == at.at_qkv)) only_here = false;
            if (o.kind == OP_ATTN && o.at_qkv == at.at_qkv) only_here = false;
            if (o.kind == OP_CAST && o.cast_src == at.at_qkv) only_here = false;
        }
        const Tensor& td = P->tensors[pr.dst];
        const bool stats = td.stats_off >= 0;
        if (!only_here || !attn_fold_shape_ok(P->dtype, P->B, tx.H * tx.W, C, stats ? C / groups : 0, stats ? td.stats_tiles : 0)) continue;
        at.at_fold_qkv = ai - 1;
        qc.folded_into = ai;
        at.fold_M = cur;
        cur = align_up(cur + (int64_t)C * C * es, 256);
        at.fold_wpv = cur;
        cur = align_up(cur + (int64_t)C * C * es, 256);
        at.fold_c = cur;
        cur = align_up(cur + (int64_t)C * 4, 256);
        at.fold_b2 = cur;
        cur = align_up(cur + (int64_t)C * 4, 256);
        AttnFoldJob jb{};
        jb.wq = P->params[qc.w].packed_off;
        jb.bq = P->params[qc.b].packed_off;
        jb.wp = P->params[pr.w].packed_off;
        jb.bp = P->params[pr.b].packed_off;
        jb.M = at.fold_M;
        jb.c = at.fold_c;
        jb.wpv = at.fold_wpv;
        jb.bias2 = at.fold_b2;
        jb.C = C;
        P->fold_jobs.push_back(jb);
        if (C > P->fold_maxC) P->fold_maxC = C;
    }
    P->packed_bytes = cur;
}

int run_gn(const dmme_plan* P, const Op& o, const char* pk, char* ws, int nt, const float* drop_masks, hipStream_t s) {
    if (o.gn_direct || o.gn_in_consumer) return DMME_OK;
    const float* tsh = o.gn_mod_col >= 0 ? (const float*)(ws + P->ws_tproj) + o.gn_mod_col : nullptr;
    const float* tsc = tsh ? tsh + o.gn_mod_C : nullptr;
    int rc;
    const Tensor& t1 = P->tensors[o.gn_src1];
    const void* s1 = ws + t1.off;
    const void* s2 = o.gn_src2 >= 0 ? ws + P->tensors[o.gn_src2].off : nullptr;
    const int C2 = o.gn_src2 >= 0 ? P->tensors[o.gn_src2].C : 0;
    const float* gam = (const float*)(pk + P->params[o.gn_gamma].packed_off);
    const float* bet = (const float*)(pk + P->params[o.gn_beta].packed_off);
    float* sc = (float*)(ws + o.gn_scale);
    float* sh = (float*)(ws + o.gn_shift);
    if (gn_from_parts(P, o)) {
        const Tensor* t2 = o.gn_src2 >= 0 ? &P->tensors[o.gn_src2] : nullptr;
        return launch_gn_finalize_parts((const float*)(ws + t1.stats_off), t1.stats_tiles, t1.stats_cnt, t1.C,
                                        t2 ? (const float*)(ws + t2->stats_off) : nullptr, t2 ? t2->stats_tiles : 0,
                                        t2 ? t2->stats_cnt : 0, C2, P->B, P->cfg.num_groups, gam, bet, 1e-5f, sc, sh,
                                        (float*)(ws + o.gn_mr), tsh, tsc, P->tproj_cols, nt, s);
    }
    const int gdt = t1.f32 ? DMME_F32 : P->dtype;
    if (gn_fast_supported(gdt, P->B, t1.H * t1.W, t1.C, C2, P->cfg.num_groups)) {
        void* act = nullptr;
        int act_silu = 0;
        const float* dm = nullptr;
        if (o.gn_act >= 0) {
            const Op& cv = P->ops[o.gn_consumer];
            act = ws + o.gn_act;
            act_silu = cv.pro_silu;
            if (cv.dmask_off >= 0 && drop_masks) dm = drop_masks + cv.dmask_off;
        }
        rc = launch_gn_fast(gdt, s1, s2, P->B, t1.H * t1.W, t1.C, C2, P->cfg.num_groups, gam, bet, 1e-5f, sc, sh,
                            (float*)(ws + o.gn_mr), (float*)(ws + P->ws_gnpart), s, act, act_silu, dm);
    }
    else
        rc = launch_gn_generic(gdt, s1, s2, P->B, t1.H * t1.W, t1.C, C2, P->cfg.num_groups, gam, bet, 1e-5f, sc, sh,
                               (float*)(ws + o.gn_mr), s);
    if (rc != DMME_OK || !tsh) return rc;
    return launch_gn_modulate(sc, sh, tsh, tsc, P->tproj_cols, nt, P->B, o.gn_mod_C, s);
}

int run_op(const dmme_plan* P, const Op& o, const char* pk, const float* x, const int64_t* t, int nt, float* y,
           char* ws, const float* drop_masks, hipStream_t s, bool keep_ctx, const int64_t* labels = nullptr, int* status = nullptr) {
    if (o.lvl >= 0) return o.lvl_first ? run_level(P, P->lvl_runs[o.lvl], pk, ws, nt, drop_masks, s, keep_ctx) : DMME_OK;
    if (o.fused_away) return DMME_OK;
    const bool fold = !keep_ctx && P->fold_packed == (const void*)pk;
    if (fold && o.kind == OP_CONV && o.folded_into >= 0) return DMME_OK;
    switch (o.kind) {
        case OP_SINUS:
            return launch_time_sinusoid(t, nt, (const float*)(pk + P->params[P->freqs_param].packed_off),
                                        P->cfg.pos_dim / 2, (float*)(ws + P->ws_tsin), s, (unsigned*)(ws + P->ws_mark),
                                        keep_ctx ? kFwdMarkKeep : kFwdMarkNograd);
        case OP_LINEAR: {
            const char* w = o.lin_w >= 0 ? pk + P->params[o.lin_w].packed_off : pk + P->tproj_w_off;
            const float* b = (const float*)(o.lin_b >= 0 ? pk + P->params[o.lin_b].packed_off : pk + P->tproj_b_off);
            if (nt > 4)
                return launch_small_gemm(P->dtype, 0, (const float*)(ws + o.lin_in), o.lin_K, w, o.lin_K, nt, o.lin_N, o.lin_K, b, o.lin_silu,
                                         (float*)(ws + o.lin_out), o.lin_N, s, o.lin_pre >= 0 ? (float*)(ws + o.lin_pre) : nullptr);
            return launch_linear_wave(P->dtype, (const float*)(ws + o.lin_in), nt, o.lin_K, w, b, o.lin_N, o.lin_silu,
                                      (float*)(ws + o.lin_out), s);
        }
        case OP_LABEL: {
            float* z2 = (float*)(ws + P->ws_tz2);
            return launch_label_cond(z2, nt, (const float*)(pk + P->params[P->p_lemb].packed_off), labels, P->B, P->cfg.num_classes, P->cfg.emb_dim,
                                     (float*)(ws + P->ws_temb), nt == P->B ? z2 : nullptr, status, s);
        }
        case OP_GN:
            return run_gn(P, o, pk, ws, nt, drop_masks, s);
        case OP_CONV: {
            ConvArgs a{};
            fill_conv(P, o, pk, x, y, ws, drop_masks, nt, a, true);
            return launch_conv(conv_dt(P, o), a, s);
        }
        case OP_CAST: {
            const Tensor& ts = P->tensors[o.cast_src];
            return launch_cast_f32_to_16(P->dtype, (const float*)(ws + ts.off), (int64_t)P->B * ts.H * ts.W * ts.C, ws + P->tensors[o.cast_dst].off, s);
        }
        case OP_ATTN: {
            const Tensor& q = P->tensors[o.at_qkv];
            const int S = q.H * q.W, C = q.C / 3;
            if (fold && o.at_fold_qkv >= 0) {
                ConvArgs a{}, qa{};
                fill_conv(P, P->ops[o.at_proj], pk, x, y, ws, drop_masks, nt, a, true);
                fill_conv(P, P->ops[o.at_fold_qkv], pk, x, y, ws, drop_masks, nt, qa, true);
                return launch_attn_fold(P->dtype, qa.src1, P->B, S, C, qa.has_gni ? &qa.gni : nullptr, qa.scale, qa.shift, pk + o.fold_M, (const float*)(pk + o.fold_c), pk + o.fold_wpv,
                                        (const float*)(pk + o.fold_b2), a.res1, a.dst, a.gn_part, a.gn_tiles, a.gn_cg, s);
            }
            if (o.at_proj >= 0) {
                ConvArgs a{};
                fill_conv(P, P->ops[o.at_proj], pk, x, y, ws, drop_masks, nt, a, true);
                return launch_attn_proj(P->dtype, ws + q.off, P->B, S, C, keep_ctx ? ws + P->tensors[o.at_out].off : nullptr, (float*)(ws + o.at_lse), a.w, a.bias,
                                        a.res1, a.dst, a.gn_part, a.gn_tiles, a.gn_cg, s);
            }
            if (P->x3 && attn_x3_supported(P->B, S, C, o.at_heads))
                return launch_attn_x3(ws + q.off, P->B, S, C, o.at_heads, ws + P->tensors[o.at_out].off, s);
            if (o.at_heads > 1) {
                if (attn_heads_mfma_supported(P->dtype, P->B, S, C, o.at_heads))
                    return launch_attn_heads_mfma(P->dtype, ws + q.off, P->B, S, C, o.at_heads, ws + P->tensors[o.at_out].off, (float*)(ws + o.at_lse), s);
                return launch_attn_heads(P->dtype, ws + q.off, P->B, S, C, o.at_heads, ws + P->tensors[o.at_out].off, s);
            }
            if (attn_mfma_supported(P->dtype, P->B, S, C))
                return launch_attn_mfma(P->dtype, ws + q.off, P->B, S, C, ws + P->tensors[o.at_out].off, (float*)(ws + o.at_lse), s);
            return launch_attn_generic(P->dtype, ws + q.off, P->B, S, C, ws + P->tensors[o.at_out].off, s);
        }
    }
    return DMME_OK;
}
void op_account(const dmme_plan* P, const Op& o, char* label, int cap, double* flops, double* bytes) {
    const double es = (double)dtype_size(P->dtype);
    const char* tn = P->dtype == DMME_BF16 ? "bf16" : P->dtype == DMME_F16 ? "f16" : "float";
    const double B = P->B;
    *flops = 0;
    *bytes = 0;
    if (o.lvl >= 0) {
        const LvlRun& R = P->lvl_runs[o.lvl];
        if (o.lvl_first) {
            snprintf(label, cap, "lvl_engine_kernel<%dx%d>", 1 << R.sh, 1 << R.sh);
            *flops = R.flops;
            *bytes = R.bytes;
        } else {
            snprintf(label, cap, "(level engine)");
        }
        return;
    }
    if (o.fused_away) {
        snprintf(label, cap, o.fused_away == 2 ? "(proj 1x1 conv inside its block's attention launch)" : "(residual 1x1 conv inside its block's conv2)");
        return;
    }
    switch (o.kind) {
        case OP_SINUS:
            snprintf(label, cap, "time_sinusoid_kernel");
            break;
        case OP_LABEL:
            snprintf(label, cap, "label_cond_kernel");
            *flops = B * P->cfg.emb_dim;
            *bytes = 4.0 * B * P->cfg.emb_dim * 3;
            break;
        case OP_LINEAR:
            snprintf(label, cap, "linear_wave_kernel<%s>", tn);
            *flops = 2.0 * o.lin_K * o.lin_N;
            *bytes = (double)o.lin_K * o.lin_N * es + 4.0 * (o.lin_K + 2.0 * o.lin_N);
            break;
        case OP_GN: {
            const Tensor& t1 = P->tensors[o.gn_src1];
            const int C = t1.C + (o.gn_src2 >= 0 ? P->tensors[o.gn_src2].C : 0);
            const bool fast = gn_fast_supported(P->dtype, P->B, t1.H * t1.W, t1.C, C - t1.C, P->cfg.num_groups);
            if (o.gn_direct || o.gn_in_consumer) {
                snprintf(label, cap, o.gn_direct ? "(norm finished by its producers' epilogues)" : "(norm finished by its consumer's parameter fill)");
            } else if (gn_from_parts(P, o)) {
                snprintf(label, cap, "gn_finalize_parts_kernel");
                *bytes = 2.0 * B * C * 4;
            } else {
                snprintf(label, cap, fast ? "gn_partial_kernel<%s>" : "gn_generic_kernel<%s>", tn);
                *bytes = B * t1.H * t1.W * C * es + 2.0 * B * C * 4;
            }
            break;
        }
        case OP_CONV: {
            ConvArgs a{};
            fill_conv(P, o, (const char*)4096, (const float*)4096, (float*)4096, (char*)4096, nullptr, 1, a, true);
            const int cdt = conv_dt(P, o);
            conv_label(conv_route(cdt, a), cdt, a, label, cap);
            const double Cin = a.C1 + a.C2, opix = B * a.Hout * a.Wout;
            *flops = 2.0 * opix * a.Cout * Cin * a.taps;
            *bytes = B * a.Hin * a.Win * Cin * (a.in_nchw ? 4.0 : es) + opix * a.Cout * (a.out_nchw ? 4.0 : es) +
                     (double)a.Cout * Cin * a.taps * es + (a.res1 ? opix * a.Cout * es : 0.0);
            if (a.r_w) {
                const double Cres = a.r_C1 + a.r_C2;
                *flops += 2.0 * opix * a.Cout * Cres;
                *bytes += opix * Cres * es + (double)a.Cout * Cres * es;
            }
            break;
        }
// ... 46 lines not shown
        DMME_REQUIRE(cfg->num_classes >= 1, DMME_ERR_INVALID, "plan_create: classifier num_classes=%d", cfg->num_classes);
        DMME_REQUIRE(cfg->channels_per_depth[cfg->num_depths - 1] <= 1024, DMME_ERR_UNSUPPORTED, "plan_create: classifier head wider than 1024 channels");
    }
    if (cfg->arch == DMME_ARCH_IDDPM) {
        DMME_REQUIRE(cfg->num_heads >= 1, DMME_ERR_INVALID, "plan_create: num_heads must be >= 1");
    }
    for (int d = 0; d < cfg->num_depths; ++d)
        DMME_REQUIRE(cfg->channels_per_depth[d] > 0 && cfg->channels_per_depth[d] % cfg->num_groups == 0,
                     DMME_ERR_INVALID, "channels_per_depth[%d]=%d not divisible by num_groups=%d", d,
                     cfg->channels_per_depth[d], cfg->num_groups);
    return DMME_OK;
}

static int check_mix_kernels(const dmme_plan* P) {
    if (!P->mix) return DMME_OK;
    for (const Op& o : P->ops) {
        if (o.kind != OP_CONV || !(o.mix || o.route_f32)) continue;
        ConvArgs a{};
        fill_conv(P, o, (const char*)4096, (const float*)4096, (float*)4096, (char*)4096, nullptr, 1, a);
        const bool ok = !o.mix || conv_route(P->dtype, a).family == (o.mix == 3 ? CONV_THIN : o.mix == 4 ? CONV1X1_SPLIT : CONV3X3_SPLIT);
        DMME_REQUIRE(ok, DMME_ERR_UNSUPPORTED, "plan_create: precision fp16r32 has no kernel for the %dx%d conv %d+%d -> %d channels on the %dx%d level (B = %d)",
                     o.taps == 9 ? 3 : 1, o.taps == 9 ? 3 : 1, a.C1, a.C2, a.Cout, a.Hout, a.Wout, P->B);
    }
    return DMME_OK;
}

static int count_launches(const dmme_plan* P, bool nograd = false) {
    int n = 0;
    for (const Op& o : P->ops) {
        if (o.fused_away || (nograd && o.folded_into >= 0)) continue;
        if (o.lvl >= 0)
            n += o.lvl_first;
        else if (o.kind == OP_GN)
            n += !(o.gn_direct || o.gn_in_consumer);
        else
            ++n;
    }
    return n;
}

#define DMME_TRY(expr)                 \
    do {                               \
        if (int rc_ = (expr)) return rc_; \
    } while (0)

static int upload_tables(dmme_plan* P) {
    DMME_CHECK_HIP(hipSetDevice(P->device));
    std::vector<PackItem> items, bitems, uitems;
    build_pack_items(P, items);
    build_pack_items_bwd(P, bitems);
    build_unpack_items(P, uitems);
    P->n_items = (int)items.size();
    P->n_items_bwd = (int)bitems.size();
    P->n_items_unpack = (int)uitems.size();
    DMME_TRY(P->items_dev.upload(items));
    DMME_TRY(P->items_bwd_dev.upload(bitems));
    DMME_TRY(P->items_unpack_dev.upload(uitems));
    DMME_TRY(P->tp_tiles_dev.upload(P->tp_tiles));
    DMME_TRY(P->col_jobs_dev.upload(P->col_jobs));
    DMME_TRY(P->bias_jobs_dev.upload(P->bias_jobs));
    if (!P->fold_jobs.empty()) DMME_TRY(P->fold_jobs_dev.upload(P->fold_jobs));
    std::vector<dmme_plan::WgGroup*> all_groups{&P->wg[0], &P->wg[1], &P->wg[2]};
    for (auto& B_ : P->gb)
        for (int k = 0; k < 3; ++k) all_groups.push_back(&B_.wg[k]);
    for (dmme_plan::WgGroup* G : all_groups) {
        if (G->jobs.empty()) continue;
        DMME_TRY(G->layers_dev.upload(G->layers));
        DMME_TRY(G->jobs_dev.upload(G->jobs));
    }
    DMME_TRY(P->err_host.alloc());
    for (LvlRun& R : P->lvl_runs) {
        DMME_TRY(R.ops_dev.upload(R.ops));
        if (R.raw_skipped > 0) DMME_TRY(R.ops_nograd_dev.upload(R.ops_nograd));
        DMME_TRY(R.sync_dev.zeroed(16 + R.ops.size() * 2 * (size_t)R.NG * LVL_NS));
    }
    return DMME_OK;
}

}

extern "C" {

DMME_API const char* dmme_last_error(void) { return g_err; }
DMME_API int dmme_version(void) { return 115; }
DMME_API int dmme_device_count(void) {
    int n = 0;
    if (hipGetDeviceCount(&n) != hipSuccess) return 0;
    return n;
}

DMME_API int dmme_unet_plan_create(const dmme_unet_cfg* cfg, int B, int H, int W, int dtype, int device, dmme_plan** out) {
    DMME_REQUIRE(cfg && out, DMME_ERR_INVALID, "plan_create: null argument");
    DMME_TRY(check_cfg(cfg, B, H, W, dtype));
    std::unique_ptr<dmme_plan> owned(new dmme_plan());
    dmme_plan* P = owned.get();
    P->cfg = *cfg;
    if (cfg->arch == DMME_ARCH_DDPM_COND) {
        P->cond = 1;
        P->cfg.arch = DMME_ARCH_DDPM;
    }
    P->B = B;
    P->H = H;
    P->W = W;
    P->x3 = dtype == DMME_BF16X3;
    P->mix = dtype == DMME_F16R32;
    P->dtype = P->x3 ? DMME_F32 : P->mix ? DMME_F16 : dtype;
    P->device = device;
    DMME_TRY(build_plan(P));
    DMME_TRY(check_mix_kernels(P));
    assign_levels(P);
    const bool fused_gn = !getenv("DMME_NO_FUSED_GN");
    if (fused_gn) assign_stats(P);
    if (fused_gn && !getenv("DMME_NO_GN_DIRECT")) assign_direct(P);
    if (!getenv("DMME_NO_PREACT")) assign_preact(P);
    if (fused_gn) assign_gn_in(P);
    assign_rseg(P);
    assign_attn_proj(P);
    assign_lvl_nograd(P);
    assign_attn_fold(P);
    P->n_launches = count_launches(P);
    P->n_launches_nograd = count_launches(P, true);
    plan_backward(P);
    if (device >= 0) DMME_TRY(upload_tables(P));
    *out = owned.release();
    return DMME_OK;
}

DMME_API void dmme_unet_plan_destroy(dmme_plan* plan) { delete plan; }

DMME_API int dmme_unet_plan_num_params(const dmme_plan* plan) { return plan ? (int)plan->params.size() : 0; }

DMME_API int dmme_unet_plan_param_info(const dmme_plan* plan, int index, char* name, int name_cap, int* ndim,
                              int64_t shape[4], int64_t* ref_offset, int* is_buffer) {
    DMME_REQUIRE(plan && index >= 0 && index < (int)plan->params.size(), DMME_ERR_INVALID, "param_info: bad index %d", index);
    const Param& p = plan->params[index];
    if (name && name_cap > 0) {
        strncpy(name, p.name.c_str(), (size_t)name_cap - 1);
        name[name_cap - 1] = 0;
    }
    if (ndim) *ndim = p.ndim;
    if (shape)
        for (int i = 0; i < 4; ++i) shape[i] = p.shape[i];
    if (ref_offset) *ref_offset = p.ref_off;
    if (is_buffer) *is_buffer = p.is_buffer ? 1 : 0;
    return DMME_OK;
}

DMME_API int64_t dmme_unet_plan_ref_numel(const dmme_plan* plan) { return plan ? plan->ref_numel : 0; }
DMME_API int64_t dmme_unet_plan_packed_bytes(const dmme_plan* plan) { return plan ? plan->packed_bytes : 0; }
DMME_API int64_t dmme_unet_plan_workspace_bytes(const dmme_plan* plan) { return plan ? plan->ws_bytes : 0; }
DMME_API int64_t dmme_unet_plan_dropmask_numel(const dmme_plan* plan) { return plan ? plan->dropmask_numel : 0; }
DMME_API int dmme_unet_plan_out_channels(const dmme_plan* plan) { return plan ? plan->out_channels : 0; }
DMME_API int dmme_unet_plan_num_launches(const dmme_plan* plan) { return plan ? plan->n_launches : 0; }
DMME_API int dmme_unet_plan_num_launches_nograd(const dmme_plan* plan) { return plan ? plan->n_launches_nograd : 0; }
DMME_API int dmme_unet_plan_num_folded(const dmme_plan* plan) { return plan ? (int)plan->fold_jobs.size() : 0; }

DMME_API int dmme_unet_pack_params(const dmme_plan* plan, const float* ref_flat, void* packed, void* stream) {
    DMME_REQUIRE(plan && ref_flat && packed, DMME_ERR_INVALID, "pack_params: null argument");
    DMME_REQUIRE(plan->items_dev, DMME_ERR_INVALID, "pack_params: plan was created without a device");
    if (plan->fold_packed == packed) plan->fold_packed = nullptr;
    return launch_pack_table(plan->dtype, plan->items_dev.get(), plan->n_items, ref_flat, packed, (hipStream_t)stream);
}

DMME_API int dmme_unet_pack_folded(const dmme_plan* plan, void* packed, void* stream) {
    DMME_REQUIRE(plan && packed, DMME_ERR_INVALID, "pack_folded: null argument");
    DMME_REQUIRE(plan->items_dev, DMME_ERR_INVALID, "pack_folded: plan was created without a device");
    if (plan->fold_jobs.empty()) return DMME_OK;
    const int rc = launch_attn_fold_weights(plan->dtype, plan->fold_jobs_dev.get(), (int)plan->fold_jobs.size(), plan->fold_maxC, packed, (hipStream_t)stream);
    if (rc == DMME_OK) plan->fold_packed = packed;
    return rc;
}

static int unet_forward_impl(const dmme_plan* plan, const void* packed, const float* x, const int64_t* t, int t_len,
                      float* y, void* workspace, const float* drop_masks, void* stream, bool keep_ctx, const int64_t* labels = nullptr,
                      int* status = nullptr) {
    DMME_REQUIRE(plan && packed && x && t && y && workspace, DMME_ERR_INVALID, "unet_forward: null argument");
    DMME_REQUIRE((plan->cond != 0) == (labels != nullptr), DMME_ERR_INVALID,
                 plan->cond ? "unet_forward: a class-conditional plan (DMME_ARCH_DDPM_COND) takes labels: call dmme_unet_forward_cond / dmme_cfg_chain_step"
                            : "unet_forward_cond: the plan is not class-conditional (DMME_ARCH_DDPM_COND)");
    DMME_REQUIRE(t_len == 1 || t_len == plan->B, DMME_ERR_INVALID,
                 "unet_forward: timestep tensor of length %d does not broadcast against batch %d", t_len, plan->B);
    {
        const int rc = lvl_check(plan, "unet_forward", (hipStream_t)stream, true);
        if (rc != DMME_OK) return rc;
    }
    hipStream_t s = (hipStream_t)stream;
    const dmme_plan* P = plan;
    const char* pk = (const char*)packed;
    char* ws = (char*)workspace;
    const int nt = t_len;
    if (keep_ctx) {
        if (plan->nograd_ws == workspace) plan->nograd_ws = nullptr;
    } else {
        plan->nograd_ws = workspace;
    }
    for (int oi = 0; oi < (int)P->ops.size(); ++oi) {
        const int rc = run_op(P, P->ops[oi], pk, x, t, P->cond && oi > P->label_op ? P->B : nt, y, ws, drop_masks, s, keep_ctx, labels, status);
        if (rc != DMME_OK) return rc;
    }
    if (P->head_src >= 0) {
        const Tensor& tt = P->tensors[P->head_src];
        return launch_cls_head_fwd(P->dtype, ws + tt.off, P->B, tt.H * tt.W, tt.C, P->cfg.num_groups, (const float*)(pk + P->params[P->p_hgw].packed_off),
                                   (const float*)(pk + P->params[P->p_hgb].packed_off), (const float*)(pk + P->params[P->p_hw].packed_off),
                                   (const float*)(pk + P->params[P->p_hb].packed_off), P->out_channels, y, s);
    }
    return DMME_OK;
}
DMME_API int dmme_unet_forward(const dmme_plan* plan, const void* packed, const float* x, const int64_t* t, int t_len,
                      float* y, void* workspace, const float* drop_masks, void* stream) {
    return unet_forward_impl(plan, packed, x, t, t_len, y, workspace, drop_masks, stream, true);
}
DMME_API int dmme_unet_forward_nograd(const dmme_plan* plan, const void* packed, const float* x, const int64_t* t, int t_len,
                      float* y, void* workspace, const float* drop_masks, void* stream) {
    return unet_forward_impl(plan, packed, x, t, t_len, y, workspace, drop_masks, stream, false);
}

DMME_API int dmme_unet_forward_cond(const dmme_plan* plan, const void* packed, const float* x, const int64_t* t, int t_len, const int64_t* labels,
                                    float* y, void* workspace, const float* drop_masks, int keep_ctx, int* status, void* stream) {
    DMME_REQUIRE(labels, DMME_ERR_INVALID, "unet_forward_cond: null argument (labels)");
    return unet_forward_impl(plan, packed, x, t, t_len, y, workspace, drop_masks, stream, keep_ctx != 0, labels, status);
}

DMME_API int dmme_unet_plan_num_ops(const dmme_plan* plan) { return plan ? (int)plan->ops.size() : 0; }

DMME_API int dmme_unet_plan_op_info(const dmme_plan* plan, int index, char* label, int label_cap, double* flops,
                                    double* bytes) {
    DMME_REQUIRE(plan && index >= 0 && index < (int)plan->ops.size() && label && label_cap > 0 && flops && bytes,
                 DMME_ERR_INVALID, "op_info: bad argument");
    op_account(plan, plan->ops[index], label, label_cap, flops, bytes);
    return DMME_OK;
}

DMME_API int dmme_unet_forward_profiled(const dmme_plan* plan, const void* packed, const float* x, const int64_t* t,
                                        int t_len, float* y, void* workspace, const float* drop_masks, void* stream,
                                        float* op_ms) {
    DMME_REQUIRE(plan && packed && x && t && y && workspace && op_ms, DMME_ERR_INVALID, "forward_profiled: null argument");
    DMME_REQUIRE(t_len == 1 || t_len == plan->B, DMME_ERR_INVALID, "forward_profiled: bad t_len %d", t_len);
    DMME_REQUIRE(!plan->cond, DMME_ERR_INVALID, "forward_profiled: a class-conditional plan takes labels (dmme_unet_forward_cond); this entry point has none");
    if (int rc0 = lvl_check(plan, "forward_profiled", (hipStream_t)stream, true)) return rc0;
    hipStream_t s = (hipStream_t)stream;
    const size_t n = plan->ops.size();
    plan->nograd_ws = workspace;
    std::vector<hipEvent_t> ev(n + 1);
    for (auto& e : ev) DMME_CHECK_HIP(hipEventCreate(&e));
    int rc = DMME_OK;
    DMME_CHECK_HIP(hipEventRecord(ev[0], s));
    for (size_t i = 0; i < n && rc == DMME_OK; ++i) {
        rc = run_op(plan, plan->ops[i], (const char*)packed, x, t, t_len, y, (char*)workspace, drop_masks, s, false);
        if (rc == DMME_OK && hipEventRecord(ev[i + 1], s) != hipSuccess) rc = DMME_ERR_HIP;
    }
    if (rc == DMME_OK && hipEventSynchronize(ev[n]) != hipSuccess) rc = DMME_ERR_HIP;
    for (size_t i = 0; i < n && rc == DMME_OK; ++i)
        if (hipEventElapsedTime(&op_ms[i], ev[i], ev[i + 1]) != hipSuccess) rc = DMME_ERR_HIP;
    for (auto& e : ev) (void)hipEventDestroy(e);
    if (rc == DMME_ERR_HIP) set_error("forward_profiled: HIP event error");
    return rc;
}

DMME_API int dmme_grad_norm(const float* grad, int64_t numel, float* norm_out, float* scratch, void* stream) {
    DMME_REQUIRE(grad && norm_out && scratch && numel > 0, DMME_ERR_INVALID, "grad_norm: bad argument");
    return launch_grad_norm(grad, numel, norm_out, scratch, (hipStream_t)stream);
}

DMME_API int dmme_adam_step(float* param, const float* grad, float* exp_avg, float* exp_avg_sq, float* ema, int64_t numel, float lr,
                            float beta1, float beta2, float eps, int step, const float* grad_norm, float max_norm, float ema_decay,
                            float grad_scale, void* stream) {
    DMME_REQUIRE(param && grad && exp_avg && exp_avg_sq && numel > 0 && step >= 1 && grad_scale > 0.f, DMME_ERR_INVALID, "adam_step: bad argument");
    return launch_adam(param, grad, exp_avg, exp_avg_sq, ema, numel, lr, beta1, beta2, eps, step, grad_norm, max_norm, ema_decay, grad_scale,
                       (hipStream_t)stream);
}

DMME_API int dmme_amp_init(float* amp_state, float init_scale, void* stream) {
    DMME_REQUIRE(amp_state && init_scale > 0.f, DMME_ERR_INVALID, "amp_init: bad argument");
    return launch_amp_init(amp_state, init_scale, (hipStream_t)stream);
}
DMME_API int dmme_amp_scale(float* grad, int64_t numel, const float* amp_state, void* stream) {
    DMME_REQUIRE(grad && amp_state && numel >= 0, DMME_ERR_INVALID, "amp_scale: bad argument");
    return launch_amp_scale(grad, numel, amp_state, (hipStream_t)stream);
}
DMME_API int dmme_adam_step_amp(float* param, const float* grad, float* exp_avg, float* exp_avg_sq, float* ema, int64_t numel, float lr, float beta1,
                                float beta2, float eps, const float* grad_norm, float max_grad_norm, float ema_decay, float grad_scale,
                                float* amp_state, float growth_factor, float backoff_factor, int growth_interval, void* stream) {
    DMME_REQUIRE(param && grad && exp_avg && exp_avg_sq && grad_norm && amp_state, DMME_ERR_INVALID, "adam_step_amp: null argument");
    DMME_REQUIRE(numel > 0 && grad_scale > 0.f, DMME_ERR_INVALID, "adam_step_amp: bad argument");
    DMME_REQUIRE(growth_factor >= 1.f && backoff_factor > 0.f && backoff_factor <= 1.f && growth_interval >= 1, DMME_ERR_INVALID, "adam_step_amp: bad scaler constants");
    return launch_adam_amp(param, grad, exp_avg, exp_avg_sq, ema, numel, lr, beta1, beta2, eps, grad_norm, max_grad_norm, ema_decay, grad_scale, amp_state,
                           growth_factor, backoff_factor, growth_interval, (hipStream_t)stream);
}

DMME_API int dmme_grad_pack_bf16(const float* grad, int64_t numel, void* dst_bf16, int64_t numel_padded, void* stream) {
    DMME_REQUIRE(grad && dst_bf16 && numel > 0 && numel_padded >= numel, DMME_ERR_INVALID, "grad_pack_bf16: bad argument");
    return launch_grad_pack_bf16(grad, numel, dst_bf16, numel_padded, (hipStream_t)stream);
}
DMME_API int dmme_shard_reduce_bf16(const void* recv_bf16, int world, int64_t per_rank, float scale, void* out_bf16, void* stream) {
    DMME_REQUIRE(recv_bf16 && out_bf16 && world >= 1 && per_rank > 0, DMME_ERR_INVALID, "shard_reduce_bf16: bad argument");
    return launch_shard_reduce_bf16(recv_bf16, world, per_rank, scale, out_bf16, (hipStream_t)stream);
}
DMME_API int dmme_grad_unpack_bf16(const void* src_bf16, int64_t numel, float* grad, void* stream) {
    DMME_REQUIRE(src_bf16 && grad && numel > 0, DMME_ERR_INVALID, "grad_unpack_bf16: bad argument");
    return launch_grad_unpack_bf16(src_bf16, numel, grad, (hipStream_t)stream);
}

DMME_API int dmme_unet_debug_read(const dmme_plan* plan, const void* workspace, const char* name, float* dst,
                         int64_t numel_cap, int64_t* numel_out, void* stream) {
    DMME_REQUIRE(plan && workspace && name && dst, DMME_ERR_INVALID, "debug_read: null argument");
    hipStream_t s = (hipStream_t)stream;
    if (strcmp(name, "condition") == 0) {
        const int64_t n = (int64_t)plan->B * plan->cfg.emb_dim;
        DMME_REQUIRE(n <= numel_cap, DMME_ERR_INVALID, "debug_read: destination too small");
        DMME_CHECK_HIP(hipMemcpyAsync(dst, (const char*)workspace + plan->ws_temb, (size_t)n * 4, hipMemcpyDeviceToDevice, s));
        if (numel_out) *numel_out = n;
        return DMME_OK;
    }
    auto it = plan->named.find(name);
    DMME_REQUIRE(it != plan->named.end(), DMME_ERR_INVALID, "debug_read: unknown module '%s'", name);
    const Tensor& t = plan->tensors[it->second];
    const int64_t n = (int64_t)plan->B * t.C * t.H * t.W;
    DMME_REQUIRE(n <= numel_cap, DMME_ERR_INVALID, "debug_read: destination too small (%lld > %lld)", (long long)n,
                 (long long)numel_cap);
    if (numel_out) *numel_out = n;
    return launch_nhwc_to_nchw(t.f32 ? DMME_F32 : plan->dtype, (const char*)workspace + t.off, plan->B, t.C, t.H * t.W, dst, s);
}

DMME_API int dmme_unet_debug_read_grad(const dmme_plan* plan, const void* bwd_workspace, const char* name, float* dst,
                                       int64_t numel_cap, int64_t* numel_out, void* stream) {
    DMME_REQUIRE(plan && bwd_workspace && name && dst, DMME_ERR_INVALID, "debug_read_grad: null argument");
    DMME_REQUIRE(strcmp(name, "condition") != 0, DMME_ERR_INVALID,
                 "debug_read_grad: the gradient of 'condition' is not kept (the time-MLP backward overwrites it in place with the gradient "
                 "of the pre-activation); compare the condition.* parameter gradients instead");
    auto it = plan->named.find(name);
    DMME_REQUIRE(it != plan->named.end(), DMME_ERR_INVALID, "debug_read_grad: unknown module '%s'", name);
    const Tensor& t = plan->tensors[it->second];
    const int64_t n = (int64_t)plan->B * t.C * t.H * t.W;
    DMME_REQUIRE(n <= numel_cap, DMME_ERR_INVALID, "debug_read_grad: destination too small (%lld > %lld)", (long long)n,
                 (long long)numel_cap);
    if (numel_out) *numel_out = n;
    return launch_nhwc_to_nchw(plan->dtype, (const char*)bwd_workspace + plan->gt_off[it->second], plan->B, t.C, t.H * t.W, dst,
                               (hipStream_t)stream);
}

DMME_API int dmme_unet_debug_read_norm_stats(const dmme_plan* plan, const void* workspace, const char* name, float* dst,
                                             int64_t numel_cap, int64_t* numel_out, void* stream) {
    DMME_REQUIRE(plan && workspace && name && dst, DMME_ERR_INVALID, "debug_read_norm_stats: null argument");
    const std::string key = std::string(name) + ".weight";
    for (const Op& o : plan->ops) {
        if (o.kind != OP_GN || o.gn_gamma < 0 || plan->params[o.gn_gamma].name != key) continue;
        const int64_t n = (int64_t)plan->B * plan->cfg.num_groups * 2;
        DMME_REQUIRE(n <= numel_cap, DMME_ERR_INVALID, "debug_read_norm_stats: destination too small (%lld > %lld)", (long long)n,
                     (long long)numel_cap);
        DMME_CHECK_HIP(hipMemcpyAsync(dst, (const char*)workspace + o.gn_mr, (size_t)n * 4, hipMemcpyDeviceToDevice, (hipStream_t)stream));
        if (numel_out) *numel_out = n;
        return DMME_OK;
    }
    set_error("debug_read_norm_stats: no GroupNorm named '%s'", name);
    return DMME_ERR_INVALID;
}

DMME_API int dmme_dropout_masks(const dmme_plan* plan, uint64_t seed, uint64_t offset, float* masks, void* stream) {
    DMME_REQUIRE(plan && masks, DMME_ERR_INVALID, "dropout_masks: null argument");
    return launch_dropmask(masks, plan->dropmask_numel, plan->cfg.dropout, seed, offset, (hipStream_t)stream);
}

DMME_API int dmme_randn(float* out, int64_t numel, uint64_t seed, uint64_t offset, void* stream) {
    DMME_REQUIRE(out && numel >= 0, DMME_ERR_INVALID, "randn: bad argument");
    return launch_randn(out, numel, seed, offset, (hipStream_t)stream);
}

DMME_API int dmme_q_sample(const float* x0, const float* z, const float* sqrt_abar, const float* sqrt_1m_abar,
                           const int64_t* t, int B, int64_t chw, float* x_t, float* target, void* stream) {
    DMME_REQUIRE(x0 && z && sqrt_abar && sqrt_1m_abar && t && x_t && B > 0 && chw > 0, DMME_ERR_INVALID, "q_sample: bad argument");
    return launch_q_sample(x0, z, sqrt_abar, sqrt_1m_abar, t, B, chw, x_t, target, (hipStream_t)stream);
}

static SamplerOperands sampler_operands(float* x, const float* out, const float* zin, int64_t B, int64_t chw, const float* grad = nullptr,
                                        float* hist = nullptr, int planes = 1, const float* known = nullptr, const float* mask = nullptr) {
    return SamplerOperands{x, out, grad, zin, hist, known, mask, chw, B * chw, (B * chw + 3) / 4, planes};
}

DMME_API int dmme_ddpm_step(float* x, const float* eps, const float* z, float inv_sqrt_alpha, float eps_coef, float sigma,
                   int add_noise, int64_t numel, void* stream) {
    DMME_REQUIRE(x && eps && (z || !add_noise), DMME_ERR_INVALID, "ddpm_step: null argument");
    const float row[4] = {inv_sqrt_alpha, eps_coef, sigma, 0.f};
    return launch_sampler_eager("ddpm_step", DMME_CHAIN_DDPM, sampler_operands(x, eps, z, 1, numel), row, add_noise, (hipStream_t)stream);
}

DMME_API int dmme_ddim_step(float* x, const float* eps, float sqrt_one_minus_abar, float sqrt_abar_prev, int64_t numel,
                   void* stream) {
    DMME_REQUIRE(x && eps, DMME_ERR_INVALID, "ddim_step: null argument");
    const float row[4] = {sqrt_one_minus_abar, sqrt_abar_prev, 0.f, 0.f};
    return launch_sampler_eager("ddim_step", DMME_CHAIN_DDIM, sampler_operands(x, eps, nullptr, 1, numel), row, 0, (hipStream_t)stream);
}

DMME_API int dmme_gddim_step(float* x, const float* eps, const float* z, float k0, float k1, float k2, int64_t numel, void* stream) {
    DMME_REQUIRE(x && eps && (z || k2 == 0.0f) && numel >= 0, DMME_ERR_INVALID, "gddim_step: null argument (z is needed where k2 != 0)");
    const float row[4] = {k0, k1, k2, 0.f};
    return launch_sampler_eager("gddim_step", DMME_CHAIN_GDDIM, sampler_operands(x, eps, z, 1, numel), row, 0, (hipStream_t)stream);
}

DMME_API int dmme_iddpm_step(float* x, const float* model_out, const float* z, float inv_sqrt_alpha, float eps_coef, float log_beta,
                             float log_beta_tilde, int add_noise, int B, int64_t chw, void* stream) {
    DMME_REQUIRE(x && model_out && (z || !add_noise) && B > 0 && chw > 0, DMME_ERR_INVALID, "iddpm_step: bad argument");
    const float row[4] = {inv_sqrt_alpha, eps_coef, log_beta, log_beta_tilde};
    return launch_sampler_eager("iddpm_step", DMME_CHAIN_IDDPM, sampler_operands(x, model_out, z, B, chw), row, add_noise, (hipStream_t)stream);
}

DMME_API int dmme_chain_set(void* state, int64_t i, const int64_t* t_table, uint64_t philox_seed, uint64_t philox_offset, void* stream) {
    DMME_REQUIRE(state && t_table && i >= 0, DMME_ERR_INVALID, "chain_set: bad argument");
    return launch_chain_set(state, i, t_table, philox_seed, philox_offset, (hipStream_t)stream);
}

DMME_API int dmme_chain_update(int kind, float* x, const float* model_out, const float* step_coef, const int64_t* t_table, void* state,
                               int B, int64_t chw, void* stream) {
    DMME_REQUIRE(x && model_out && step_coef && t_table && state && B > 0 && chw > 0, DMME_ERR_INVALID, "chain_update: bad argument");
    DMME_REQUIRE(kind >= DMME_CHAIN_DDPM && kind <= DMME_CHAIN_GDDIM, DMME_ERR_INVALID, "chain_update: unknown sampler kind %d", kind);
    return launch_sampler_chain("chain_update", kind, sampler_operands(x, model_out, nullptr, B, chw), step_coef, t_table, state, (hipStream_t)stream);
}

DMME_API int dmme_chain_update_gddim(float* x, const float* model_out, const float* noise, const float* step_coef, const int64_t* t_table,
                                     void* state, int B, int64_t chw, void* stream) {
    DMME_REQUIRE(x && model_out && step_coef && t_table && state && B > 0 && chw > 0, DMME_ERR_INVALID, "chain_update_gddim: bad argument");
    return launch_sampler_chain("chain_update_gddim", DMME_CHAIN_GDDIM, sampler_operands(x, model_out, noise, B, chw), step_coef, t_table, state,
                                (hipStream_t)stream);
}

DMME_API int dmme_chain_update_guided(int kind, float* x, const float* model_out, const float* grad, const float* noise, const float* step_coef,
                                      const int64_t* t_table, void* state, int B, int64_t chw, void* stream) {
    DMME_REQUIRE(x && model_out && grad && step_coef && t_table && state && B > 0 && chw > 0, DMME_ERR_INVALID, "chain_update_guided: bad argument");
    DMME_REQUIRE(kind_grad(kind), DMME_ERR_INVALID, "chain_update_guided: kind %d is not a guided kind", kind);
    return launch_sampler_chain("chain_update_guided", kind, sampler_operands(x, model_out, noise, B, chw, grad), step_coef, t_table, state,
                                (hipStream_t)stream);
}

static bool kind_plain_cfg(int kind) { return kind == DMME_CHAIN_DDPM_CFG || kind == DMME_CHAIN_GDDIM_CFG; }
DMME_API int dmme_cfg_step(int kind, float* x, const float* model_out, const float* z, float c0, float c1, float c2, float s, int add_noise, int B,
                           int64_t chw, void* stream) {
    DMME_REQUIRE(kind_plain_cfg(kind), DMME_ERR_INVALID, "cfg_step: kind %d is not a classifier-free kind (6, 7)", kind);
    const float row[4] = {c0, c1, c2, s};
    return launch_sampler_eager("cfg_step", kind, sampler_operands(x, model_out, z, B, chw), row, add_noise, (hipStream_t)stream);
}

DMME_API int dmme_chain_update_cfg(int kind, float* x, const float* model_out, const float* noise, const float* step_coef, const int64_t* t_table,
                                   void* state, int B, int64_t chw, void* stream) {
    DMME_REQUIRE(kind_plain_cfg(kind), DMME_ERR_INVALID, "chain_update_cfg: kind %d is not a classifier-free kind (6, 7)", kind);
    return launch_sampler_chain("chain_update_cfg", kind, sampler_operands(x, model_out, noise, B, chw), step_coef, t_table, state, (hipStream_t)stream);
}

DMME_API int dmme_dpmpp_step(float* x, const float* model_out, float* history, const float* row, int history_valid, int B, int64_t chw, int out_planes,
                             void* stream) {
    return launch_sampler_eager("dpmpp_step", DMME_CHAIN_DPMPP, sampler_operands(x, model_out, nullptr, B, chw, nullptr, history, out_planes), row,
                                history_valid, (hipStream_t)stream);
}

DMME_API int dmme_chain_update_dpmpp(float* x, const float* model_out, float* history, const float* step_coef, const int64_t* t_table, void* state, int B,
                                     int64_t chw, int out_planes, void* stream) {
    return launch_sampler_chain("chain_update_dpmpp", DMME_CHAIN_DPMPP, sampler_operands(x, model_out, nullptr, B, chw, nullptr, history, out_planes),
                                step_coef, t_table, state, (hipStream_t)stream);
}

DMME_API int dmme_cfg_dpmpp_step(float* x_2B, const float* model_out, float* history, const float* row, int history_valid, int B, int64_t chw, void* stream) {
    return launch_sampler_eager("cfg_dpmpp_step", DMME_CHAIN_DPMPP_CFG, sampler_operands(x_2B, model_out, nullptr, B, chw, nullptr, history), row, history_valid,
                                (hipStream_t)stream);
}

DMME_API int dmme_chain_update_cfg_dpmpp(float* x_2B, const float* model_out, float* history, const float* step_coef, const int64_t* t_table, void* state,
                                         int B, int64_t chw, void* stream) {
    return launch_sampler_chain("chain_update_cfg_dpmpp", DMME_CHAIN_DPMPP_CFG, sampler_operands(x_2B, model_out, nullptr, B, chw, nullptr, history), step_coef,
                                t_table, state, (hipStream_t)stream);
}

DMME_API int dmme_repaint_step(float* x, const float* model_out, const float* known, const float* mask, const float* z3, const float* row, int B,
                               int64_t chw, int out_planes, void* stream) {
    return launch_sampler_eager("repaint_step", DMME_CHAIN_REPAINT, sampler_operands(x, model_out, z3, B, chw, nullptr, nullptr, out_planes, known, mask), row, 0,
                                (hipStream_t)stream);
}

DMME_API int dmme_chain_update_repaint(float* x, const float* model_out, const float* known, const float* mask, const float* noise,
                                       const float* step_coef, const int64_t* t_table, void* state, int B, int64_t chw, int out_planes, void* stream) {
    return launch_sampler_chain("chain_update_repaint", DMME_CHAIN_REPAINT, sampler_operands(x, model_out, noise, B, chw, nullptr, nullptr, out_planes, known, mask),
                                step_coef, t_table, state, (hipStream_t)stream);
}

static int chain_step_common(const char* what, const dmme_plan* plan, const void* packed, float* x, const int64_t* labels, int* status, float* model_out,
                             void* workspace, int kind, const float* grad, float* hist, const float* step_coef, const int64_t* t_table, void* state,
                             void* stream, const std::function<int()>& between = nullptr, const float* known = nullptr, const float* mask = nullptr) {
    const bool cfg = kind_cfg(kind);
    DMME_REQUIRE(plan && packed && x && model_out && workspace && step_coef && t_table && state && (labels || !cfg) && (hist || !kind_hist(kind)) &&
                     ((known && mask) || !kind_paint(kind)),
                 DMME_ERR_INVALID, "%s: null argument", what);
    if (cfg)
        DMME_REQUIRE(plan->cond && plan->B % 2 == 0, DMME_ERR_INVALID,
                     "%s: needs a class-conditional plan (DMME_ARCH_DDPM_COND) of even batch: conditional half, unconditional half (B = %d)", what, plan->B);
    else
        DMME_REQUIRE(!plan->cond, DMME_ERR_INVALID, "%s: a class-conditional plan takes labels: call dmme_cfg_chain_step / dmme_cfg_dpmpp_chain_step", what);
    DMME_REQUIRE(plan->cfg.arch != DMME_ARCH_CLASSIFIER, DMME_ERR_INVALID, "%s: architecture %d predicts no noise", what, plan->cfg.arch);
    const int planes = plan->out_channels / plan->cfg.in_channels;
    DMME_REQUIRE(plan->out_channels == planes * plan->cfg.in_channels && (kind_planes(kind) ? planes == kind_planes(kind) : planes == 1 || planes == 2),
                 DMME_ERR_INVALID, "%s: sampler kind %d does not fit a network with %d output channels for %d input channels", what, kind, plan->out_channels,
                 plan->cfg.in_channels);
    if (!cfg)
        if (int rc = lvl_check(plan, what, (hipStream_t)stream, true)) return rc;
    const int64_t* t_dev = (const int64_t*)state + 1;
    if (int rc = unet_forward_impl(plan, packed, x, t_dev, 1, model_out, workspace, nullptr, stream, false, labels, status)) return rc;
    if (plan->pred != DMME_PRED_EPS)
        if (int rc = launch_pred_to_eps(plan->pred, model_out, x, plan->pred_ab, plan->pred_T, t_dev, 1, plan->B,
                                        (int64_t)plan->cfg.in_channels * plan->H * plan->W, (hipStream_t)stream))
            return rc;
    if (plan->thr_mode != DMME_THRESHOLD_NONE)
        if (int rc = launch_x0_threshold(plan->thr_mode, model_out, x, plan->thr_table, plan->thr_T, t_dev, 1, cfg ? plan->B / 2 : plan->B,
                                         (int64_t)plan->cfg.in_channels * plan->H * plan->W, planes, cfg ? 2 : 1, 1.0f, cfg ? step_coef : nullptr, kind_row(kind),
                                         kind_scol(kind), (const int64_t*)state, plan->thr_k, plan->thr_frac, plan->thr_scratch, (hipStream_t)stream))
            return rc;
    if (between)
        if (int rc = between()) return rc;
    return launch_sampler_chain(what, kind, sampler_operands(x, model_out, nullptr, cfg ? plan->B / 2 : plan->B, (int64_t)plan->cfg.in_channels * plan->H * plan->W,
                                                             grad, hist, planes, known, mask),
                                step_coef, t_table, state, (hipStream_t)stream);
}

DMME_API int dmme_chain_step(const dmme_plan* plan, const void* packed, float* x, float* model_out, void* workspace, int kind,
                             const float* step_coef, const int64_t* t_table, void* state, void* stream) {
    DMME_REQUIRE(kind_known(kind) && !kind_cfg(kind) && !kind_grad(kind) && !kind_hist(kind) && !kind_paint(kind), DMME_ERR_INVALID,
                 "chain_step: sampler kind %d (guided kinds: dmme_guided_chain_step, and so on)", kind);
    return chain_step_common("chain_step", plan, packed, x, nullptr, nullptr, model_out, workspace, kind, nullptr, nullptr, step_coef, t_table, state, stream);
}

DMME_API int dmme_cfg_chain_step(const dmme_plan* plan_2B, const void* packed, float* x_2B, const int64_t* labels_2B, float* model_out, void* workspace,
                                 int* status, int kind, const float* step_coef, const int64_t* t_table, void* state, void* stream) {
    DMME_REQUIRE(kind_plain_cfg(kind), DMME_ERR_INVALID, "cfg_chain_step: kind %d is not a classifier-free kind (6, 7)", kind);
    return chain_step_common("cfg_chain_step", plan_2B, packed, x_2B, labels_2B, status, model_out, workspace, kind, nullptr, nullptr, step_coef, t_table, state,
                             stream);
}

DMME_API int dmme_dpmpp_chain_step(const dmme_plan* plan, const void* packed, float* x, float* model_out, void* workspace, float* history,
                                   const float* step_coef, const int64_t* t_table, void* state, void* stream) {
    return chain_step_common("dpmpp_chain_step", plan, packed, x, nullptr, nullptr, model_out, workspace, DMME_CHAIN_DPMPP, nullptr, history, step_coef, t_table,
                             state, stream);
}

DMME_API int dmme_cfg_dpmpp_chain_step(const dmme_plan* plan_2B, const void* packed, float* x_2B, const int64_t* labels_2B, float* model_out, void* workspace,
                                       int* status, float* history, const float* step_coef, const int64_t* t_table, void* state, void* stream) {
    return chain_step_common("cfg_dpmpp_chain_step", plan_2B, packed, x_2B, labels_2B, status, model_out, workspace, DMME_CHAIN_DPMPP_CFG, nullptr, history,
                             step_coef, t_table, state, stream);
}

DMME_API int dmme_repaint_chain_step(const dmme_plan* plan, const void* packed, float* x, float* model_out, void* workspace, const float* known,
                                     const float* mask, const float* step_coef, const int64_t* t_table, void* state, void* stream) {
    return chain_step_common("repaint_chain_step", plan, packed, x, nullptr, nullptr, model_out, workspace, DMME_CHAIN_REPAINT, nullptr, nullptr, step_coef, t_table,
                             state, stream, nullptr, known, mask);
}

DMME_API int dmme_guided_chain_step(const dmme_plan* plan, const void* packed, const dmme_plan* cls, const void* cls_packed,
                                    const void* cls_packed_bwd, float* x, float* model_out, void* workspace, void* cls_workspace,
                                    void* cls_bwd_workspace, const int64_t* y, float* logits, float* d_logits, float* grad, int* status,
                                    int kind, const float* step_coef, const int64_t* t_table, void* state, void* stream) {
    DMME_REQUIRE(plan && packed && cls && cls_packed && cls_packed_bwd && x && model_out && workspace && cls_workspace && cls_bwd_workspace && y &&
                 logits && d_logits && grad && step_coef && t_table && state, DMME_ERR_INVALID, "guided_chain_step: null argument");
    DMME_REQUIRE(kind_grad(kind), DMME_ERR_INVALID, "guided_chain_step: kind %d is not a guided kind", kind);
    DMME_REQUIRE(plan->cfg.arch == DMME_ARCH_DDPM && !plan->cond && cls->cfg.arch == DMME_ARCH_CLASSIFIER, DMME_ERR_INVALID,
                 "guided_chain_step: needs a DDPM UNet plan and a classifier plan (got architectures %d, %d)", plan->cfg.arch, cls->cfg.arch);
    DMME_REQUIRE(plan->B == cls->B && plan->H == cls->H && plan->W == cls->W && plan->cfg.in_channels == cls->cfg.in_channels, DMME_ERR_INVALID,
                 "guided_chain_step: the UNet plan (B=%d %dx%d) and the classifier plan (B=%d %dx%d) differ", plan->B, plan->H, plan->W, cls->B, cls->H, cls->W);
    const int64_t* t_dev = (const int64_t*)state + 1;
    return chain_step_common("guided_chain_step", plan, packed, x, nullptr, nullptr, model_out, workspace, kind, grad, nullptr, step_coef, t_table, state, stream, [&] {
        int rc = unet_forward_impl(cls, cls_packed, x, t_dev, 1, logits, cls_workspace, nullptr, stream, true);
        if (rc == DMME_OK) rc = launch_log_softmax_grad(logits, y, cls->B, cls->out_channels, 1, 1.0f, nullptr, d_logits, status, (hipStream_t)stream);
        if (rc == DMME_OK)
            rc = dmme_unet_backward_input(cls, cls_packed, cls_packed_bwd, x, t_dev, 1, d_logits, cls_workspace, cls_bwd_workspace, nullptr, grad, stream);
        return rc;
    });
}

DMME_API int dmme_label_dropout(const int64_t* labels, int B, int K, float p, uint64_t seed, uint64_t offset, int64_t* out, int* status, void* stream) {
    return launch_label_dropout(labels, B, K, p, seed, offset, out, status, (hipStream_t)stream);
}

DMME_API int dmme_slerp(const float* xa, const float* xb, const float* w, int n, int B, int64_t chw, float* out, void* stream) {
    DMME_REQUIRE(xa && xb && w && out, DMME_ERR_INVALID, "slerp: null argument");
    DMME_REQUIRE(n > 0 && B > 0 && B <= 65535 && chw > 0, DMME_ERR_INVALID, "slerp: n = %d weights, B = %d images of %lld values", n, B, (long long)chw);
    DMME_REQUIRE(chw % 4 == 0, DMME_ERR_INVALID, "slerp: image size %lld is not a multiple of 4", (long long)chw);
    static std::mutex mu;
    static std::map<int, std::pair<float*, size_t>> scratch;
    const size_t need = (size_t)3 * B * slerp_parts(chw);
    float* buf = nullptr;
    {
        std::lock_guard<std::mutex> lock(mu);
        int dev = 0;
        DMME_CHECK_HIP(hipGetDevice(&dev));
        auto& e = scratch[dev];
        if (e.second < need) {
            if (e.first) DMME_CHECK_HIP(hipFree(e.first));
            e = {nullptr, 0};
            const size_t cap = need < 4096 ? 4096 : need;
            DMME_CHECK_HIP(hipMalloc((void**)&e.first, cap * sizeof(float)));
            e.second = cap;
        }
        buf = e.first;
    }
    return launch_slerp(xa, xb, w, n, B, chw, out, buf, (hipStream_t)stream);
}
// ... 240 lines not shown
```

### diffusion-models-made-easy_amd/csrc/plan_lvl.hip

```cpp
#include "plan.h"

using namespace dmme;

namespace dmme {

static int op_level(const dmme_plan* P, const Op& o) {
    auto hw = [&](int id, int& H, int& W) {
        if (id < 0) return true;
        const Tensor& t = P->tensors[id];
        if (H == 0) {
            H = t.H;
            W = t.W;
            return true;
        }
        return t.H == H && t.W == W;
    };
    int H = 0, W = 0;
    bool ok = true;
    if (o.kind == OP_CONV) {
        if (o.src1 < 0 || o.dst < 0 || o.stride != 1 || o.up || (o.taps != 1 && o.taps != 9)) return 0;
        for (int id : {o.src1, o.src2, o.dst, o.res1, o.res2}) ok = ok && hw(id, H, W);
    } else if (o.kind == OP_GN) {
        ok = hw(o.gn_src1, H, W) && hw(o.gn_src2, H, W);
    } else if (o.kind == OP_ATTN) {
// ... 259 lines not shown
                R.NGS = nb < slots ? nb : slots;
                const int max_iter = debug_route("lvl_max_iter", 2);
                if ((nb + slots - 1) / slots > max_iter) {
                    i = j;
                    continue;
                }
                P->ws_bytes = ws;
                for (const LvlXAttach& xa : xattach) {
                    LvlOp& host = P->lvl_runs[xa.run].ops[xa.op];
                    host.norm[host.n_norm++] = xa.norm;
                }
                for (auto& mk : R.made) made[mk.first] = {(int)P->lvl_runs.size(), mk.second};
                const int ri = (int)P->lvl_runs.size();
                for (int oi = i; oi < j; ++oi) {
                    Op& o = P->ops[oi];
                    o.lvl = ri;
                    o.lvl_first = oi == i;
                    if (o.kind == OP_GN) o.gn_direct = 1;
                }
                for (auto& ga : gn_acts) {
                    Op& g = P->ops[ga.first];
                    g.gn_act = ga.second;
                    for (int ci = ga.first + 1; ci < j; ++ci)
                        if (P->ops[ci].kind == OP_CONV && P->ops[ci].gn == ga.first) {
                            g.gn_consumer = ci;
                            P->ops[ci].use_act = 1;
                        }
                }
                P->lvl_runs.push_back(std::move(R));
            }
        }
        i = j;
    }
}

void assign_lvl_nograd(dmme_plan* P) {
    if (P->lvl_runs.empty()) return;
    std::vector<char> need(P->tensors.size(), 0);
    auto mark = [&](int id) { if (id >= 0) need[id] = 1; };
    for (const Op& q : P->ops) {
        if (q.kind == OP_CONV) {
            if (!(q.gn >= 0 && q.use_act)) { mark(q.src1); mark(q.src2); }
            mark(q.res1);
            mark(q.res2);
        } else if (q.kind == OP_GN) {
            for (int id : {q.gn_src1, q.gn_src2}) {
                if (id < 0) continue;
                if (q.lvl < 0) { need[id] = 1; continue; }
                for (const LvlOp& lo : P->lvl_runs[q.lvl].ops)
                    if (lo.kind == LVL_NORM && lo.dst_off == P->tensors[id].off) need[id] = 1;
            }
        } else if (q.kind == OP_ATTN) {
            if (q.lvl < 0) mark(q.at_qkv);
        } else if (q.kind == OP_CAST) {
            mark(q.cast_src);
        }
    }
    for (const auto& kv : P->named) mark(kv.second);
    std::unordered_map<int64_t, char> need_off;
    for (size_t t = 0; t < P->tensors.size(); ++t) {
        auto it = need_off.find(P->tensors[t].off);
        if (it == need_off.end()) need_off[P->tensors[t].off] = need[t];
        else it->second = it->second || need[t];
    }
    const bool keep_all = debug_route("lvl_keep_raw") != 0;
    for (LvlRun& R : P->lvl_runs) {
        R.ops_nograd = R.ops;
        R.raw_skipped = 0;
        if (keep_all) continue;
        for (LvlOp& lo : R.ops_nograd) {
            if (lo.kind != LVL_CONV || lo.dst_off < 0) continue;
            auto it = need_off.find(lo.dst_off);
            if (it != need_off.end() && !it->second && (lo.n_norm > 0 || lo.keep >= 0)) {
                lo.dst_off = -1;
                ++R.raw_skipped;
            }
        }
    }
}

static long long* g_lvl_stamps = nullptr;
static int g_lvl_stamp_run = -1, g_lvl_stamp_wg = 0;

int run_level(const dmme_plan* P, const LvlRun& R, const char* pk, char* ws, int nt, const float* drop_masks, hipStream_t s, bool keep_ctx) {
    DMME_REQUIRE(R.ops_dev && R.sync_dev, DMME_ERR_INVALID, "level engine: the plan was created without a device");
    LvlArgs a{};
    a.ops = (!keep_ctx && R.ops_nograd_dev) ? R.ops_nograd_dev.get() : R.ops_dev.get();
    a.n_ops = (int)R.ops.size();
    a.ws = ws;
    a.packed = pk;
    a.drop_masks = drop_masks;
    a.tproj = (const float*)(ws + P->ws_tproj);
    a.tproj_ld = P->tproj_cols;
    a.nt = nt;
    a.N = P->B;
    a.sh = R.sh;
    a.NG = R.NG;
    a.NGS = R.NGS;
    a.GB = R.GB;
    a.NJ = R.NJ;
    a.ctl = R.sync_dev.get();
    a.flags = R.sync_dev.get() + 16;
    a.err_sys = P->err_host.get();
    a.run_tag = 1 + (int)(&R - P->lvl_runs.data());
    a.spin_limit = debug_route("lvl_spin", 0);
    a.withhold = debug_route("lvl_withhold", 0);
    a.xcd_group = debug_route("lvl_no_xcd") ? 0 : 1;
    a.max_wg = P->lvl_max_wg;
    if (g_lvl_stamps && g_lvl_stamp_run == (int)(&R - P->lvl_runs.data())) {
        a.stamps = g_lvl_stamps;
        a.stamp_wg = g_lvl_stamp_wg;
    }
    return launch_lvl_engine(P->dtype, a, s);
}

int lvl_check(const dmme_plan* P, const char* where, hipStream_t stream, bool have_stream) {
    if (!P->err_host) return DMME_OK;
    const unsigned v = __atomic_load_n(P->err_host.get(), __ATOMIC_ACQUIRE);
    if (!v) return DMME_OK;
    hipStreamCaptureStatus cs = hipStreamCaptureStatusNone;
    if (have_stream && hipStreamIsCapturing(stream, &cs) != hipSuccess) cs = hipStreamCaptureStatusNone;
    if (cs == hipStreamCaptureStatusNone) {
        int cur = -1;
        const bool sw = hipGetDevice(&cur) == hipSuccess && cur != P->device && hipSetDevice(P->device) == hipSuccess;
        (void)hipDeviceSynchronize();
        for (const LvlRun& R : P->lvl_runs)
            if (R.sync_dev) (void)hipMemset(R.sync_dev.get() + 2, 0, 4);
        __atomic_store_n(P->err_host.get(), 0u, __ATOMIC_RELEASE);
        if (sw) (void)hipSetDevice(cur);
    }
    if (v == kErrNogradBackward) {
        set_error("%s: a dmme_unet_backward ran on a workspace whose last forward was the no-grad form (a replayed graph of "
                  "dmme_unet_forward_nograd / dmme_chain_step, which leave out the tensors only a backward pass reads): that backward's "
                  "gradients are NaN.  Run dmme_unet_forward before dmme_unet_backward.", where);
        return DMME_ERR_INVALID;
    }
    const int ri = (int)v - 1;
    const LvlRun* R = ri >= 0 && ri < (int)P->lvl_runs.size() ? &P->lvl_runs[ri] : nullptr;
    set_error("%s: a hand-off wait of the level engine timed out (run %d, %dx%d maps, %d workgroups that must all be resident at once; the device "
              "holds %d): every output of this plan since the last check is invalid.  Typical cause: compute units held by another stream / "
              "process / CU mask.  DMME_NO_LVL=1 selects the per-op kernels.",
              where, ri, R ? 1 << R->sh : 0, R ? 1 << R->sh : 0, R ? R->NGS * (LVL_NS / R->NJ) : 0, P->lvl_max_wg);
    return DMME_ERR_HIP;
}

}

extern "C" {

DMME_API int dmme_unet_plan_check(const dmme_plan* plan) {
    DMME_REQUIRE(plan, DMME_ERR_INVALID, "plan_check: null plan");
    return lvl_check(plan, "plan_check");
}

DMME_API int dmme_unet_plan_level_info(const dmme_plan* plan, char* buf, int cap) {
    DMME_REQUIRE(plan && buf && cap > 0, DMME_ERR_INVALID, "level_info: bad argument");
    std::string out;
    char tmp[192];
    snprintf(tmp, sizeof(tmp), "runs=%d", (int)plan->lvl_runs.size());
    out = tmp;
    for (const LvlRun& R : plan->lvl_runs) {
        unsigned ctl[3] = {0, 0, 0};
        if (R.sync_dev) DMME_CHECK_HIP(hipMemcpy(ctl, R.sync_dev.get(), sizeof(ctl), hipMemcpyDeviceToHost));
        snprintf(tmp, sizeof(tmp), " [map=%dx%d plan_ops=%d-%d engine_ops=%d groups=%d per_iteration=%d slice=%d workgroups=%d nograd_raw_skipped=%d epoch=%u err=%u]", 1 << R.sh, 1 << R.sh,
                 R.op_first, R.op_last, (int)R.ops.size(), R.NG, R.GB, 32 * R.NJ, R.NGS * (LVL_NS / R.NJ), R.raw_skipped, ctl[0], ctl[2]);
        out += tmp;
    }
    strncpy(buf, out.c_str(), (size_t)cap - 1);
    buf[cap - 1] = 0;
    return DMME_OK;
}

DMME_API int dmme_debug_level_stamps(void* buf, int run, int workgroup) {
    g_lvl_stamps = (long long*)buf;
    g_lvl_stamp_run = run;
// ... 5 lines not shown
```

### diffusion-models-made-easy_amd/diffusion_models/chain.py

```python

from __future__ import annotations

import gc
from typing import Optional

import torch
from torch import Tensor

from .. import _lib
from ..common import vis
from ..common.noise import philox_reserve


class ChainTables:

    def __init__(self, rows, ttab, device):
        self.coef = torch.tensor(rows, dtype=torch.float32).reshape(-1).to(device)
        self.ttab = torch.tensor(ttab, dtype=torch.int64).to(device)
        self.state = torch.zeros(8, dtype=torch.int64, device=device)

    def set(self, i: int, seed: int = 0, offset: int = 0):
        _lib.check(_lib.lib().dmme_chain_set(_lib.ptr(self.state), int(i), _lib.ptr(self.ttab), seed & 0xFFFFFFFFFFFFFFFF, int(offset), _lib.stream_ptr()), "dmme_chain_set")


# ... 37 lines not shown
            raise ValueError(f"HistoryRecorder: ordinal {self.ordinals[-1]} in a chain of {count} steps")
        self.recorded = 0

    def at(self, s: int, x: Tensor) -> None:
        k = self._slot.get(s)
        if k is not None:
            vis.grid_tile(x[: self.n_images], self.canvas, k, self.stride, self.xmaps, self.ymaps, self.pad)
            self.recorded += 1


def walk(x: Tensor, first: int, count: int, step, recorder=None, reserve=None) -> Tensor:
    if recorder is not None:
        recorder.begin(x, count)
    if reserve is not None:
        reserve()
    for s in range(count):
        if recorder is not None:
            recorder.at(s, x)
        step(s, first - s)
    if recorder is not None:
        recorder.at(count, x)
    return x


def capture(launch, check, carried=()):
    saved = [b.clone() for b in carried]

    def restore():
        for b, v in zip(carried, saved):
            b.copy_(v)

    launch()
    torch.cuda.synchronize()
    check()
    restore()
    graph, out, error = None, None, None
    gc.collect()
    gc_was_on = gc.isenabled()
    gc.disable()
    try:
        graph = torch.cuda.CUDAGraph()
        with torch.cuda.graph(graph):
            out = launch()
    except RuntimeError as exc:
        graph, out, error = None, None, exc
    finally:
        if gc_was_on:
            gc.enable()
    restore()
    return graph, out, error


class ChainRunner(ChainTables):

    def __init__(self, process, x: Tensor, use_graph: bool = True, spec=None):
        model = process.model
        if not (isinstance(x, Tensor) and x.is_cuda and x.dtype == torch.float32 and x.is_contiguous() and x.dim() == 4):
            raise ValueError("ChainRunner needs a contiguous fp32 GPU image batch")
        B, _, H, W = x.shape
        self.process, self.model, self.x = process, model, x
        self.plan = model._plan_for(B, H, W, x.device)
        self.kind, (n, rows, ttab) = spec if spec is not None else (process._chain_kind, process._chain_tables())
        self.draws = chain_draws(self.kind, rows)
        self.n_steps = n
        self.pred = getattr(process, "_pred", _lib.PRED_EPS)
        self.pred_ab = process._pred_table(x.device).clone() if self.pred != _lib.PRED_EPS else None
        self.thr = getattr(process, "_thr", _lib.THRESHOLD_NONE)
        self.thr_tab, self.thr_scratch, self.thr_k, self.thr_frac = None, None, 0, 0.0
        if self.thr != _lib.THRESHOLD_NONE:
            from .ddpm import threshold_rank

            self.thr_tab = process._thr_table(x.device).clone()
            if self.thr == _lib.THRESHOLD_DYNAMIC:
                self.thr_k, self.thr_frac = threshold_rank(process.threshold_percentile, x[0].numel())
                self.thr_scratch = torch.empty(int(_lib.lib().dmme_x0_threshold_scratch_bytes(B, x[0].numel())) // 4, dtype=torch.int32, device=x.device)
        super().__init__(rows, ttab, x.device)
        self.out =torch.empty((B, model.out_channels, H, W), dtype=torch.float32, device=x.device)
        self.quads = x.numel() // 4
        self.noise_numel = x.numel()
        self.use_graph = use_graph
        self.graph = None
        self.capture_error = None
        self._wkey = None

    def _set_prediction(self, plan=None):
        plan = self.plan if plan is None else plan
        _lib.check(_lib.lib().dmme_unet_plan_set_prediction(plan.h, self.pred, _lib.ptr(self.pred_ab), self.process.timesteps), "dmme_unet_plan_set_prediction")

    def no_threshold(self):
        self.thr = _lib.THRESHOLD_NONE
        return self

    def _set_threshold(self, plan=None):
        plan = self.plan if plan is None else plan
        _lib.check(_lib.lib().dmme_unet_plan_set_threshold(plan.h, self.thr, _lib.ptr(self.thr_tab), self.process.timesteps, self.thr_k, self.thr_frac,
                                                           _lib.ptr(self.thr_scratch)), "dmme_unet_plan_set_threshold")

    def _launch(self, packed):
        self._set_prediction()
        self._set_threshold()
        self._call(packed)
        self.plan.overwritten()

    def _call(self, packed):
        _lib.check(
            _lib.lib().dmme_chain_step(self.plan.h, _lib.ptr(packed), _lib.ptr(self.x), _lib.ptr(self.out), _lib.ptr(self.plan.workspace), self.kind,
                                       _lib.ptr(self.coef), _lib.ptr(self.ttab), _lib.ptr(self.state), _lib.stream_ptr()),
            "dmme_chain_step",
        )

    def _carried(self):
        return [self.x, self.state]

    def _weights_key(self):
        return (self.plan.packed_version, self.plan.fold_version, self.plan.packed.data_ptr())

    def step(self):
        model = self.model
        if model.training:
            raise RuntimeError("ChainRunner: sampling chains run in eval mode (no dropout masks inside the replayed step)")
        packed = model._packed_for(self.plan, fold=True)
        wkey = self._weights_key()
        if not self.use_graph or self.capture_error is not None:
            self._launch(packed)
            return self.x
        if self.graph is None or self._wkey != wkey:
            self.graph, _, self.capture_error = capture(lambda: self._launch(packed), self.plan.check, self._carried())
            if self.graph is None:
                self._launch(packed)
                return self.x
            self._wkey = wkey
        self.plan.check()
        self.graph.replay()
        self.plan.overwritten()
        return self.x

    def run(self, first: int, count: int, recorder: Optional[HistoryRecorder] = None):

        def reserve():
            seed, off = philox_reserve(self.x.device, self.noise_numel * count) if self.draws else (0, 0)
            self.set(first, seed, off)

        walk(self.x, first, count, lambda s, i: self.step(), recorder, reserve)
        torch.cuda.current_stream(self.x.device).synchronize()
        self.plan.check()
        return self.x
```

### include/dmme_hip.h

```cpp
#ifndef DMME_HIP_H
#define DMME_HIP_H

#include <stddef.h>
#include <stdint.h>

#if defined(DMME_BUILD)
#define DMME_API __attribute__((visibility("default")))
#else
#define DMME_API
#endif

#ifdef __cplusplus
extern "C" {
#endif

typedef enum {
    DMME_OK = 0,
    DMME_ERR_INVALID = -1,
    DMME_ERR_UNSUPPORTED = -2,
    DMME_ERR_HIP = -3,
    DMME_ERR_NOMEM = -4
} dmme_status;

typedef enum { DMME_F32 = 0, DMME_BF16 = 1, DMME_BF16X3 = 2, DMME_F16 = 3, DMME_F16R32 = 4 } dmme_dtype;
// ... 87 lines not shown
DMME_API int dmme_debug_mfma_valu(int mode, int iters, int blocks, void* sink, void* stream);
DMME_API int dmme_debug_issue_probe(int kind, int n_inner, int iters, int flags, int blocks, void* sink, const void* src, void* stream);
DMME_API int dmme_debug_l2_stream(const void* buf, int64_t bytes, int iters, int mode, int depth, int blocks, void* sink, void* stream);
DMME_API int dmme_grad_norm(const float* grad, int64_t numel, float* norm_out, float* scratch, void* stream);
DMME_API int dmme_adam_step(float* param, const float* grad, float* exp_avg, float* exp_avg_sq, float* ema, int64_t numel,
                            float lr, float beta1, float beta2, float eps, int step, const float* grad_norm, float max_norm,
                            float ema_decay, float grad_scale, void* stream);
DMME_API int dmme_amp_init(float* amp_state, float init_scale, void* stream);
DMME_API int dmme_amp_scale(float* grad, int64_t numel, const float* amp_state, void* stream);
DMME_API int dmme_adam_step_amp(float* param, const float* grad, float* exp_avg, float* exp_avg_sq, float* ema, int64_t numel, float lr, float beta1,
                                float beta2, float eps, const float* grad_norm, float max_grad_norm, float ema_decay, float grad_scale,
                                float* amp_state, float growth_factor, float backoff_factor, int growth_interval, void* stream);
DMME_API int dmme_grad_pack_bf16(const float* grad, int64_t numel, void* dst_bf16, int64_t numel_padded, void* stream);
DMME_API int dmme_shard_reduce_bf16(const void* recv_bf16, int world, int64_t per_rank, float scale, void* out_bf16, void* stream);
DMME_API int dmme_grad_unpack_bf16(const void* src_bf16, int64_t numel, float* grad, void* stream);

DMME_API int dmme_unet_debug_read(const dmme_plan* plan, const void* workspace, const char* name, float* dst,
                         int64_t numel_cap, int64_t* numel_out, void* stream);
DMME_API int dmme_unet_debug_read_grad(const dmme_plan* plan, const void* bwd_workspace, const char* name, float* dst,
                         int64_t numel_cap, int64_t* numel_out, void* stream);
DMME_API int dmme_unet_debug_read_norm_stats(const dmme_plan* plan, const void* workspace, const char* name, float* dst,
                         int64_t numel_cap, int64_t* numel_out, void* stream);


DMME_API int dmme_dropout_masks(const dmme_plan* plan, uint64_t seed, uint64_t offset, float* masks, void* stream);


DMME_API int dmme_randn(float* out, int64_t numel, uint64_t seed, uint64_t offset, void* stream);

DMME_API int dmme_q_sample(const float* x0, const float* z, const float* sqrt_abar, const float* sqrt_1m_abar,
                  const int64_t* t, int B, int64_t chw, float* x_t, float* target, void* stream);

DMME_API int dmme_ddpm_step(float* x, const float* eps, const float* z, float inv_sqrt_alpha, float eps_coef,
                   float sigma, int add_noise, int64_t numel, void* stream);

DMME_API int dmme_ddim_step(float* x, const float* eps, float sqrt_one_minus_abar, float sqrt_abar_prev, int64_t numel,
                   void* stream);

DMME_API int dmme_gddim_step(float* x, const float* eps, const float* z, float k0, float k1, float k2, int64_t numel, void* stream);

DMME_API int dmme_slerp(const float* xa, const float* xb, const float* w, int n, int B, int64_t chw, float* out, void* stream);

DMME_API int dmme_mse_loss(const float* eps, const float* target, int64_t numel, float* loss, float* d_eps,
                  float grad_scale, float* scratch, void* stream);

enum { DMME_PRED_EPS = 0, DMME_PRED_X0 = 1, DMME_PRED_V = 2 };

DMME_API int dmme_pred_to_eps(int pred, float* model_out, const float* x, const float* ab, int T, const int64_t* t, int t_len, int B,
                              int64_t chw, void* stream);

DMME_API int dmme_unet_plan_set_prediction(dmme_plan* plan, int pred, const float* ab, int T);

enum { DMME_THRESHOLD_NONE = 0, DMME_THRESHOLD_STATIC = 1, DMME_THRESHOLD_DYNAMIC = 2 };

DMME_API int dmme_x0_threshold(int mode, float* model_out, const float* x, const float* table, int T, const int64_t* t, int t_len, int B,
                               int64_t chw, int planes, int halves, float guidance_scale, int k, float frac, void* scratch, void* stream);
DMME_API int64_t dmme_x0_threshold_scratch_bytes(int B, int64_t chw);
DMME_API int dmme_x0_threshold_lds_capacity(void);

DMME_API int dmme_unet_plan_set_threshold(dmme_plan* plan, int mode, const float* table, int T, int k, float frac, void* scratch);

DMME_API int dmme_q_sample_pred(int pred, const float* x0, const float* z, const float* sqrt_abar, const float* sqrt_1m_abar, const int64_t* t,
                                int B, int64_t chw, float* x_t, float* target, void* stream);

DMME_API int dmme_mse_loss_rows(const float* out, const float* target, const float* w_table, const int64_t* t, int B, int64_t chw, float* loss,
                                float* d_out, float grad_scale, float* scratch, void* stream);

DMME_API int dmme_image_batch(const uint8_t* data, int64_t n_images, const int64_t* idx, const uint8_t* flip, int B, int C, int H, int W,
                     float* out, void* stream);

DMME_API int dmme_grid_tile(const float* x, int B, int C, int H, int W, int cell0, int cell_stride, int xmaps, int ymaps, int pad, int out_kind,
                   int raw, void* canvas, void* stream);

enum { DMME_CHAIN_DDPM = 0, DMME_CHAIN_DDIM = 1, DMME_CHAIN_IDDPM = 2, DMME_CHAIN_DDPM_GUIDED = 3, DMME_CHAIN_DDIM_GUIDED = 4, DMME_CHAIN_GDDIM = 5,
       DMME_CHAIN_DDPM_CFG = 6, DMME_CHAIN_GDDIM_CFG = 7  };
DMME_API int dmme_chain_set(void* state, int64_t i, const int64_t* t_table, uint64_t philox_seed, uint64_t philox_offset, void* stream);
DMME_API int dmme_chain_update(int kind, float* x, const float* model_out, const float* step_coef, const int64_t* t_table, void* state,
                      int B, int64_t chw, void* stream);
DMME_API int dmme_chain_step(const dmme_plan* plan, const void* packed, float* x, float* model_out, void* workspace, int kind,
                    const float* step_coef, const int64_t* t_table, void* state, void* stream);
DMME_API int dmme_chain_update_gddim(float* x, const float* model_out, const float* noise, const float* step_coef, const int64_t* t_table,
                            void* state, int B, int64_t chw, void* stream);

DMME_API int dmme_log_softmax_grad(const float* logits, const int64_t* y, int B, int K, int mode, float scale, float* loss, float* d_logits,
                                   int* status, void* stream);
DMME_API int dmme_chain_update_guided(int kind, float* x, const float* model_out, const float* grad, const float* noise, const float* step_coef,
                                      const int64_t* t_table, void* state, int B, int64_t chw, void* stream);
DMME_API int dmme_guided_chain_step(const dmme_plan* plan, const void* packed, const dmme_plan* cls, const void* cls_packed,
                                    const void* cls_packed_bwd, float* x, float* model_out, void* workspace, void* cls_workspace,
                                    void* cls_bwd_workspace, const int64_t* y, float* logits, float* d_logits, float* grad, int* status,
                                    int kind, const float* step_coef, const int64_t* t_table, void* state, void* stream);

DMME_API int dmme_label_dropout(const int64_t* labels, int B, int K, float p, uint64_t seed, uint64_t offset, int64_t* out, int* status, void* stream);
DMME_API int dmme_cfg_step(int kind, float* x, const float* model_out, const float* z, float c0, float c1, float c2, float s, int add_noise, int B,
                           int64_t chw, void* stream);
DMME_API int dmme_chain_update_cfg(int kind, float* x, const float* model_out, const float* noise, const float* step_coef, const int64_t* t_table,
                                   void* state, int B, int64_t chw, void* stream);
DMME_API int dmme_cfg_chain_step(const dmme_plan* plan_2B, const void* packed, float* x_2B, const int64_t* labels_2B, float* model_out, void* workspace,
                                 int* status, int kind, const float* step_coef, const int64_t* t_table, void* state, void* stream);

enum { DMME_CHAIN_DPMPP = 8, DMME_CHAIN_DPMPP_CFG = 9 };
DMME_API int dmme_dpmpp_step(float* x, const float* model_out, float* history, const float* row, int history_valid, int B, int64_t chw, int out_planes,
                             void* stream);
DMME_API int dmme_chain_update_dpmpp(float* x, const float* model_out, float* history, const float* step_coef, const int64_t* t_table, void* state, int B,
                                     int64_t chw, int out_planes, void* stream);
DMME_API int dmme_dpmpp_chain_step(const dmme_plan* plan, const void* packed, float* x, float* model_out, void* workspace, float* history,
                                   const float* step_coef, const int64_t* t_table, void* state, void* stream);
DMME_API int dmme_cfg_dpmpp_step(float* x_2B, const float* model_out, float* history, const float* row, int history_valid, int B, int64_t chw, void* stream);
DMME_API int dmme_chain_update_cfg_dpmpp(float* x_2B, const float* model_out, float* history, const float* step_coef, const int64_t* t_table, void* state,
                                         int B, int64_t chw, void* stream);
DMME_API int dmme_cfg_dpmpp_chain_step(const dmme_plan* plan_2B, const void* packed, float* x_2B, const int64_t* labels_2B, float* model_out, void* workspace,
                                       int* status, float* history, const float* step_coef, const int64_t* t_table, void* state, void* stream);

enum { DMME_CHAIN_REPAINT = 10 };
DMME_API int dmme_repaint_step(float* x, const float* model_out, const float* known, const float* mask, const float* z3, const float* row, int B,
                               int64_t chw, int out_planes, void* stream);
DMME_API int dmme_chain_update_repaint(float* x, const float* model_out, const float* known, const float* mask, const float* noise,
                                       const float* step_coef, const int64_t* t_table, void* state, int B, int64_t chw, int out_planes, void* stream);
DMME_API int dmme_repaint_chain_step(const dmme_plan* plan, const void* packed, float* x, float* model_out, void* workspace, const float* known,
                                     const float* mask, const float* step_coef, const int64_t* t_table, void* state, void* stream);


DMME_API int dmme_iddpm_step(float* x, const float* model_out, const float* z, float inv_sqrt_alpha, float eps_coef, float log_beta,
                    float log_beta_tilde, int add_noise, int B, int64_t chw, void* stream);

DMME_API int dmme_iddpm_loss(const float* model_out, const float* x_t, const float* x_0, const float* target, const int64_t* t,
                    const float* coef, int B, int64_t chw, float w_simple, float w_vlb, float* loss, float* d_out,
                    float grad_scale, float* scratch, void* stream);


DMME_API int dmme_iddpm_loss_rows(const float* model_out, const float* x_t, const float* x_0, const float* target, const int64_t* t,
                                  const float* coef, int T, const float* weight, int B, int64_t chw, float w_simple, float w_vlb, float* loss,
                                  float* rows, float* d_out, float grad_scale, int* status, float* scratch, void* stream);

DMME_API int dmme_iddpm_prior_rows(const float* x_0, int B, int64_t chw, float alpha_bar_T, float* prior, void* stream);

DMME_API int dmme_tsampler_draw(const float* hist, const int* count, int T, int H, float uniform_prob, uint64_t philox_seed,
                                uint64_t philox_offset, int B, int64_t* t, float* weight, float* p, void* stream);

DMME_API int dmme_tsampler_update(float* hist, int* count, int T, int H, const int64_t* t, const float* L, int B, int* status, void* stream);

typedef struct {
    int dtype;
    int N, Hin, Win;
    int C1, C2;
    int upsample;
    int stride;
    int taps;
    int Cout;
    int pro_silu;
    int out_silu;
    int nt;
    int tproj_ld;
    int in_nchw;
    int out_nchw;
    int force_generic;
} dmme_conv_desc;

DMME_API int dmme_conv2d(const dmme_conv_desc* d, const void* src1, const void* src2, const void* weight,
                const float* bias, const float* scale, const float* shift, const float* dmask,
                const float* tproj, const void* res1, const void* res2, int R1, void* dst, void* stream);

DMME_API int dmme_conv2d_res(const dmme_conv_desc* d, const void* src1, const void* src2, const void* weight, const float* bias,
                const float* scale, const float* shift, const float* dmask, const void* r_src1, const void* r_src2, int r_C1,
                int r_C2, const void* r_weight, const float* r_bias, void* dst, void* stream);

// ... 31 lines not shown
```

Before: 471.5 denoising steps/s (one step = UNet forward + DDPM update on a batch of 128), summed over GPUs.

## Precompute time-embedding projection rows for all sampler timesteps

Adds a table that holds the time-embedding MLP and per-block time-projection outputs for every timestep in the sampling schedule. The table is computed once per weight version. The chain step then skips the sinusoidal and linear ops in the UNet forward and reads the current row, which the chain kernel copies into a small buffer as it advances the step index. This removes several small kernels from each denoising step, at the cost of extra memory, a per-step row copy, and cache invalidation logic tied to the packed weights.

```diff
diff --git a/diffusion-models-made-easy_amd/_lib.py b/diffusion-models-made-easy_amd/_lib.py
--- a/diffusion-models-made-easy_amd/_lib.py
+++ b/diffusion-models-made-easy_amd/_lib.py
@@ -143,6 +143,12 @@
     "dmme_chain_update": (_i, [_i, _vp, _vp, _vp, _vp, _vp, _i, _i64, _vp]),
     "dmme_chain_step": (_i, [_vp, _vp, _vp, _vp, _vp, _i, _vp, _vp, _vp, _vp]),
     "dmme_chain_update_gddim": (_i, [_vp, _vp, _vp, _vp, _vp, _vp, _i, _i64, _vp]),
+    "dmme_unet_plan_time_cols": (_i, [_vp]),
+    "dmme_unet_plan_time_rows_bytes": (_i64, [_vp, _i64]),
+    "dmme_unet_time_rows_scratch_bytes": (_i64, [_vp, _i64]),
+    "dmme_unet_time_rows": (_i, [_vp, _vp, _vp, _i64, _vp, _vp, _vp]),
+    "dmme_unet_plan_set_time_rows": (_i, [_vp, _vp, _i64, _vp]),
+    "dmme_chain_set_rows": (_i, [_vp, _i64, _vp, _u64, _u64, _vp, _i64, _i, _vp, _vp]),
     "dmme_log_softmax_grad": (_i, [_vp, _vp, _i, _i, _i, _f, _vp, _vp, _vp, _vp]),
     "dmme_chain_update_guided": (_i, [_i, _vp, _vp, _vp, _vp, _vp, _vp, _vp, _i, _i64, _vp]),
     "dmme_guided_chain_step": (_i, [_vp, _vp, _vp, _vp, _vp, _vp, _vp, _vp, _vp, _vp, _vp, _vp, _vp, _vp, _vp, _i, _vp, _vp, _vp, _vp]),
diff --git a/diffusion-models-made-easy_amd/csrc/common.h b/diffusion-models-made-easy_amd/csrc/common.h
--- a/diffusion-models-made-easy_amd/csrc/common.h
+++ b/diffusion-models-made-easy_amd/csrc/common.h
@@ -363,7 +363,13 @@
                         hipStream_t s);
 int slerp_parts(int64_t chw);
 int launch_slerp(const float* xa, const float* xb, const float* w, int n, int B, int64_t chw, float* out, float* scratch, hipStream_t s);
-int launch_chain_set(void* state, int64_t i, const int64_t* t_table, uint64_t seed, uint64_t offset, hipStream_t s);
+struct ChainRows {
+    const float* table;
+    float* cur;
+    unsigned* mark;
+    int cols;
+};
+int launch_chain_set(void* state, int64_t i, const int64_t* t_table, uint64_t seed, uint64_t offset, hipStream_t s, const ChainRows* rows = nullptr);
 
 constexpr bool kind_known(int k) { return k >= DMME_CHAIN_DDPM && k <= DMME_CHAIN_REPAINT; }
 constexpr bool kind_cfg(int k) { return k == DMME_CHAIN_DDPM_CFG || k == DMME_CHAIN_GDDIM_CFG || k == DMME_CHAIN_DPMPP_CFG; }
@@ -400,7 +406,8 @@
     int planes;
 };
 int launch_sampler_eager(const char* what, int kind, const SamplerOperands& o, const float* row, int flag, hipStream_t s);
-int launch_sampler_chain(const char* what, int kind, const SamplerOperands& o, const float* coef, const int64_t* t_table, void* state, hipStream_t s);
+int launch_sampler_chain(const char* what, int kind, const SamplerOperands& o, const float* coef, const int64_t* t_table, void* state, hipStream_t s,
+                         const ChainRows* rows = nullptr);
 int launch_label_dropout(const int64_t* labels, int B, int K, float p, uint64_t seed, uint64_t offset, int64_t* out, int* status, hipStream_t s);
 int launch_cls_head_fwd(int dtype, const void* top, int B, int HW, int C, int G, const float* gamma, const float* beta, const float* W,
                         const float* bias, int K, float* logits, hipStream_t s);
diff --git a/diffusion-models-made-easy_amd/csrc/kernels_sampler.hip b/diffusion-models-made-easy_amd/csrc/kernels_sampler.hip
--- a/diffusion-models-made-easy_amd/csrc/kernels_sampler.hip
+++ b/diffusion-models-made-easy_amd/csrc/kernels_sampler.hip
@@ -167,32 +167,52 @@
 };
 static_assert(sizeof(ChainState) == 64, "ChainState is eight 64-bit words (dmme_hip.h: dmme_chain_*)");
 
-__global__ void chain_set_kernel(ChainState* st, long long i, const long long* __restrict__ t_table, unsigned long long seed, unsigned long long offset) {
-    st->i = i;
-    st->t = t_table[i];
-    st->offset = offset;
-    st->seed = seed;
-    st->ticket = 0u;
-    st->pad = 0u;
-    st->history_valid = 0ull;
-}
-int launch_chain_set(void* state, int64_t i, const int64_t* t_table, uint64_t seed, uint64_t offset, hipStream_t s) {
-    hipLaunchKernelGGL(chain_set_kernel, dim3(1), dim3(1), 0, s, (ChainState*)state, (long long)i, (const long long*)t_table, (unsigned long long)seed,
-                       (unsigned long long)offset);
+__device__ __forceinline__ void chain_load_row(const ChainRows& rows, long long row, int first, int stride) {
+    const float* src = rows.table + row * rows.cols;
+    if (rows.cols % 4 == 0) {
+        for (int c = first; c < rows.cols / 4; c += stride) reinterpret_cast<float4*>(rows.cur)[c] = reinterpret_cast<const float4*>(src)[c];
+    } else {
+        for (int c = first; c < rows.cols; c += stride) rows.cur[c] = src[c];
+    }
+}
+
+__global__ void __launch_bounds__(256) chain_set_kernel(ChainState* st, long long i, const long long* __restrict__ t_table, unsigned long long seed,
+                                                        unsigned long long offset, ChainRows rows) {
+    if (i < 0) {
+        chain_load_row(rows, st->i, threadIdx.x, blockDim.x);
+        return;
+    }
+    if (threadIdx.x == 0) {
+        st->i = i;
+        st->t = t_table[i];
+        st->offset = offset;
+        st->seed = seed;
+        st->ticket = 0u;
+        st->pad = 0u;
+        st->history_valid = 0ull;
+    }
+    if (rows.cur) chain_load_row(rows, i, threadIdx.x, blockDim.x);
+}
+int launch_chain_set(void* state, int64_t i, const int64_t* t_table, uint64_t seed, uint64_t offset, hipStream_t s, const ChainRows* rows) {
+    DMME_REQUIRE(i >= 0 || rows, DMME_ERR_INVALID, "chain_set: a negative index reloads the time row of a chain that has one");
+    hipLaunchKernelGGL(chain_set_kernel, dim3(1), dim3(rows ? 256 : 1), 0, s, (ChainState*)state, (long long)i, (const long long*)t_table,
+                       (unsigned long long)seed, (unsigned long long)offset, rows ? *rows : ChainRows{});
     DMME_CHECK_LAUNCH();
     return DMME_OK;
 }
 
 __device__ __forceinline__ void chain_advance(ChainState* st, const long long* __restrict__ t_table, long long i, unsigned long long offset_inc,
-                                              bool raise_history) {
+                                              bool raise_history, const ChainRows& rows) {
+    const long long ni = i > 0 ? i - 1 : 0;
+    if (rows.cur) chain_load_row(rows, ni, blockIdx.x * blockDim.x + threadIdx.x, gridDim.x * blockDim.x);
     if (threadIdx.x != 0) return;
     const unsigned tk = atomicAdd(&st->ticket, 1u);
     if (tk != gridDim.x - 1) return;
-    const long long ni = i > 0 ? i - 1 : 0;
     st->i = ni;
     st->t = t_table[ni];
     if (offset_inc) st->offset += offset_inc;
     if (raise_history) st->history_valid = 1ull;
+    if (rows.mark) *rows.mark = kFwdMarkNograd;
     atomicExch(&st->ticket, 0u);
 }
 
@@ -284,7 +304,7 @@
 }
 
 template <int KIND>
-__global__ void __launch_bounds__(256) __attribute__((amdgpu_waves_per_eu(8))) chain_kernel(SamplerOperands o, const float* __restrict__ coef, const long long* __restrict__ t_table, ChainState* st) {
+__global__ void __launch_bounds__(256) __attribute__((amdgpu_waves_per_eu(8))) chain_kernel(SamplerOperands o, const float* __restrict__ coef, const long long* __restrict__ t_table, ChainState* st, ChainRows rows) {
     const long long i = st->i, t = st->t;
     const unsigned long long off = st->offset, seed = st->seed;
     Row r;
@@ -297,7 +317,7 @@
         update_quad<KIND>(o, q, r, flag, z);
     }
     __syncthreads();
-    chain_advance(st, t_table, i, kind_hist(KIND) ? 0ull : (unsigned long long)o.n4 * kind_streams(KIND), kind_hist(KIND));
+    chain_advance(st, t_table, i, kind_hist(KIND) ? 0ull : (unsigned long long)o.n4 * kind_streams(KIND), kind_hist(KIND), rows);
 }
 
 template <int K = 0, class F>
@@ -339,11 +359,13 @@
         }
     });
 }
-int launch_sampler_chain(const char* what, int kind, const SamplerOperands& o, const float* coef, const int64_t* t_table, void* state, hipStream_t s) {
+int launch_sampler_chain(const char* what, int kind, const SamplerOperands& o, const float* coef, const int64_t* t_table, void* state, hipStream_t s,
+                         const ChainRows* rows) {
     if (int rc = check_operands(what, kind, o, false)) return rc;
     DMME_REQUIRE(coef && t_table && state, DMME_ERR_INVALID, "%s: null argument", what);
+    const ChainRows cr = rows ? *rows : ChainRows{};
     return dispatch_kind(kind, [&](auto k) -> int {
-        hipLaunchKernelGGL(chain_kernel<decltype(k)::value>, dim3(grid_for(o.n4)), dim3(256), 0, s, o, coef, (const long long*)t_table, (ChainState*)state);
+        hipLaunchKernelGGL(chain_kernel<decltype(k)::value>, dim3(grid_for(o.n4)), dim3(256), 0, s, o, coef, (const long long*)t_table, (ChainState*)state, cr);
         DMME_CHECK_LAUNCH();
         return DMME_OK;
     });
diff --git a/diffusion-models-made-easy_amd/csrc/plan.h b/diffusion-models-made-easy_amd/csrc/plan.h
--- a/diffusion-models-made-easy_amd/csrc/plan.h
+++ b/diffusion-models-made-easy_amd/csrc/plan.h
@@ -221,6 +221,9 @@
     float thr_frac = 0.f;
     const float* thr_table = nullptr;
     void* thr_scratch = nullptr;
+    const float* trow_table = nullptr;
+    float* trow_cur = nullptr;
+    int64_t trow_n = 0;
 };
 
 namespace dmme {
@@ -229,12 +232,15 @@
 static inline int conv_dt(const dmme_plan* P, const Op& o) { return o.route_f32 ? DMME_F32 : P->dtype; }
 static inline int wg_index(const Op& o) { return o.taps == 1 ? 1 : o.stride == 2 ? 2 : 0; }
 
+static inline const float* tproj_rows(const dmme_plan* P, const char* ws, const float* trow) { return trow ? trow : (const float*)(ws + P->ws_tproj); }
+
 void fill_conv(const dmme_plan* P, const Op& o, const char* packed, const float* x, float* y, char* ws, const float* drop_masks, int nt, ConvArgs& a,
-               bool fwd = false);
+               bool fwd = false, const float* trow = nullptr);
 bool gn_from_parts(const dmme_plan* P, const Op& o);
 void assign_levels(dmme_plan* P);
 void assign_rseg(dmme_plan* P);
-int run_level(const dmme_plan* P, const LvlRun& R, const char* pk, char* ws, int nt, const float* drop_masks, hipStream_t s, bool keep_ctx = true);
+int run_level(const dmme_plan* P, const LvlRun& R, const char* pk, char* ws, int nt, const float* drop_masks, hipStream_t s, bool keep_ctx = true,
+              const float* trow = nullptr);
 void assign_lvl_nograd(dmme_plan* P);
 void assign_attn_fold(dmme_plan* P);
 int lvl_check(const dmme_plan* P, const char* where, hipStream_t stream = nullptr, bool have_stream = false);
diff --git a/diffusion-models-made-easy_amd/csrc/plan.hip b/diffusion-models-made-easy_amd/csrc/plan.hip
--- a/diffusion-models-made-easy_amd/csrc/plan.hip
+++ b/diffusion-models-made-easy_amd/csrc/plan.hip
@@ -576,7 +576,7 @@
 }
 
 void fill_conv(const dmme_plan* P, const Op& o, const char* packed, const float* x, float* y, char* ws,
-               const float* drop_masks, int nt, ConvArgs& a, bool fwd) {
+               const float* drop_masks, int nt, ConvArgs& a, bool fwd, const float* trow) {
     const int64_t es = (int64_t)dtype_size(P->dtype);
     (void)es;
     a.x3 = P->x3 || o.route_f32;
@@ -633,7 +633,7 @@
             a.gni.eps = 1e-5f;
             a.gni.mean_rstd = (float*)(ws + g.gn_mr);
             if (g.gn_mod_col >= 0) {
-                a.gni.t_shift = (const float*)(ws + P->ws_tproj) + g.gn_mod_col;
+                a.gni.t_shift = tproj_rows(P, ws, trow) + g.gn_mod_col;
                 a.gni.t_scale = a.gni.t_shift + g.gn_mod_C;
                 a.gni.t_ld = P->tproj_cols;
                 a.gni.nt = nt;
@@ -652,7 +652,7 @@
         a.pro_silu = 0;
     }
     if (o.tproj_col >= 0) {
-        a.tproj = (const float*)(ws + P->ws_tproj) + o.tproj_col;
+        a.tproj = tproj_rows(P, ws, trow) + o.tproj_col;
         a.tproj_ld = P->tproj_cols;
         a.nt = nt;
     }
@@ -997,9 +997,9 @@
     P->packed_bytes = cur;
 }
 
-int run_gn(const dmme_plan* P, const Op& o, const char* pk, char* ws, int nt, const float* drop_masks, hipStream_t s) {
+int run_gn(const dmme_plan* P, const Op& o, const char* pk, char* ws, int nt, const float* drop_masks, hipStream_t s, const float* trow = nullptr) {
     if (o.gn_direct || o.gn_in_consumer) return DMME_OK;
-    const float* tsh = o.gn_mod_col >= 0 ? (const float*)(ws + P->ws_tproj) + o.gn_mod_col : nullptr;
+    const float* tsh = o.gn_mod_col >= 0 ? tproj_rows(P, ws, trow) + o.gn_mod_col : nullptr;
     const float* tsc = tsh ? tsh + o.gn_mod_C : nullptr;
     int rc;
     const Tensor& t1 = P->tensors[o.gn_src1];
@@ -1039,8 +1039,10 @@
 }
 
 int run_op(const dmme_plan* P, const Op& o, const char* pk, const float* x, const int64_t* t, int nt, float* y,
-           char* ws, const float* drop_masks, hipStream_t s, bool keep_ctx, const int64_t* labels = nullptr, int* status = nullptr) {
-    if (o.lvl >= 0) return o.lvl_first ? run_level(P, P->lvl_runs[o.lvl], pk, ws, nt, drop_masks, s, keep_ctx) : DMME_OK;
+           char* ws, const float* drop_masks, hipStream_t s, bool keep_ctx, const int64_t* labels = nullptr, int* status = nullptr,
+           const float* trow = nullptr) {
+    if (o.lvl >= 0) return o.lvl_first ? run_level(P, P->lvl_runs[o.lvl], pk, ws, nt, drop_masks, s, keep_ctx, trow) : DMME_OK;
+    if (trow && (o.kind == OP_SINUS || o.kind == OP_LINEAR)) return DMME_OK;
     if (o.fused_away) return DMME_OK;
     const bool fold = !keep_ctx && P->fold_packed == (const void*)pk;
     if (fold && o.kind == OP_CONV && o.folded_into >= 0) return DMME_OK;
@@ -1064,10 +1066,10 @@
                                      (float*)(ws + P->ws_temb), nt == P->B ? z2 : nullptr, status, s);
         }
         case OP_GN:
-            return run_gn(P, o, pk, ws, nt, drop_masks, s);
+            return run_gn(P, o, pk, ws, nt, drop_masks, s, trow);
         case OP_CONV: {
             ConvArgs a{};
-            fill_conv(P, o, pk, x, y, ws, drop_masks, nt, a, true);
+            fill_conv(P, o, pk, x, y, ws, drop_masks, nt, a, true, trow);
             return launch_conv(conv_dt(P, o), a, s);
         }
         case OP_CAST: {
@@ -1079,14 +1081,14 @@
             const int S = q.H * q.W, C = q.C / 3;
             if (fold && o.at_fold_qkv >= 0) {
                 ConvArgs a{}, qa{};
-                fill_conv(P, P->ops[o.at_proj], pk, x, y, ws, drop_masks, nt, a, true);
-                fill_conv(P, P->ops[o.at_fold_qkv], pk, x, y, ws, drop_masks, nt, qa, true);
+                fill_conv(P, P->ops[o.at_proj], pk, x, y, ws, drop_masks, nt, a, true, trow);
+                fill_conv(P, P->ops[o.at_fold_qkv], pk, x, y, ws, drop_masks, nt, qa, true, trow);
                 return launch_attn_fold(P->dtype, qa.src1, P->B, S, C, qa.has_gni ? &qa.gni : nullptr, qa.scale, qa.shift, pk + o.fold_M, (const float*)(pk + o.fold_c), pk + o.fold_wpv,
                                         (const float*)(pk + o.fold_b2), a.res1, a.dst, a.gn_part, a.gn_tiles, a.gn_cg, s);
             }
             if (o.at_proj >= 0) {
                 ConvArgs a{};
-                fill_conv(P, P->ops[o.at_proj], pk, x, y, ws, drop_masks, nt, a, true);
+                fill_conv(P, P->ops[o.at_proj], pk, x, y, ws, drop_masks, nt, a, true, trow);
                 return launch_attn_proj(P->dtype, ws + q.off, P->B, S, C, keep_ctx ? ws + P->tensors[o.at_out].off : nullptr, (float*)(ws + o.at_lse), a.w, a.bias,
                                         a.res1, a.dst, a.gn_part, a.gn_tiles, a.gn_cg, s);
             }
@@ -1299,7 +1301,7 @@
 extern "C" {
 
 DMME_API const char* dmme_last_error(void) { return g_err; }
-DMME_API int dmme_version(void) { return 115; }
+DMME_API int dmme_version(void) { return 116; }
 DMME_API int dmme_device_count(void) {
     int n = 0;
     if (hipGetDeviceCount(&n) != hipSuccess) return 0;
@@ -1388,10 +1390,69 @@
     return rc;
 }
 
+DMME_API int dmme_unet_plan_time_cols(const dmme_plan* plan) { return plan ? plan->tproj_cols : 0; }
+
+DMME_API int64_t dmme_unet_plan_time_rows_bytes(const dmme_plan* plan, int64_t n_rows) {
+    if (!plan || n_rows <= 0 || n_rows > (1 << 20) || plan->cond || plan->cfg.arch == DMME_ARCH_CLASSIFIER || plan->tproj_cols <= 0) return 0;
+    if (getenv("DMME_NO_TIME_ROWS") || debug_route("no_time_rows")) return 0;
+    const int64_t bytes = n_rows * plan->tproj_cols * 4;
+    return bytes > plan->packed_bytes ? 0 : bytes;
+}
+DMME_API int64_t dmme_unet_time_rows_scratch_bytes(const dmme_plan* plan, int64_t n_rows) {
+    return plan && n_rows > 0 ? n_rows * (plan->cfg.pos_dim + 2 * (int64_t)plan->cfg.emb_dim) * 4 : 0;
+}
+
+DMME_API int dmme_unet_time_rows(const dmme_plan* plan, const void* packed, const int64_t* t_table, int64_t n_rows, float* table, void* scratch,
+                                 void* stream) {
+    DMME_REQUIRE(plan && packed && t_table && table && scratch, DMME_ERR_INVALID, "time_rows: null argument");
+    DMME_REQUIRE(n_rows > 0 && n_rows <= (1 << 20), DMME_ERR_INVALID, "time_rows: %lld rows", (long long)n_rows);
+    DMME_REQUIRE(!plan->cond, DMME_ERR_UNSUPPORTED, "time_rows: the rows of a class-conditional plan depend on the label");
+    const dmme_plan* P = plan;
+    const char* pk = (const char*)packed;
+    hipStream_t s = (hipStream_t)stream;
+    const int nt = (int)n_rows;
+    float* tsin = (float*)scratch;
+    float* th1 = tsin + n_rows * P->cfg.pos_dim;
+    float* temb = th1 + n_rows * P->cfg.emb_dim;
+    auto at = [&](int64_t ws_off) -> float* {
+        return ws_off == P->ws_tsin ? tsin : ws_off == P->ws_th1 ? th1 : ws_off == P->ws_temb ? temb : ws_off == P->ws_tproj ? table : nullptr;
+    };
+    for (const Op& o : P->ops) {
+        if (o.kind == OP_SINUS) {
+            DMME_TRY(launch_time_sinusoid(t_table, nt, (const float*)(pk + P->params[P->freqs_param].packed_off), P->cfg.pos_dim / 2, tsin, s));
+        } else if (o.kind == OP_LINEAR) {
+            const float* in = at(o.lin_in);
+            float* out = at(o.lin_out);
+            DMME_REQUIRE(in && out, DMME_ERR_INVALID, "time_rows: a linear op outside the time path");
+            const char* w = o.lin_w >= 0 ? pk + P->params[o.lin_w].packed_off : pk + P->tproj_w_off;
+            const float* b = (const float*)(o.lin_b >= 0 ? pk + P->params[o.lin_b].packed_off : pk + P->tproj_b_off);
+            DMME_TRY(launch_linear_wave(P->dtype, in, nt, o.lin_K, w, b, o.lin_N, o.lin_silu, out, s));
+        }
+    }
+    return DMME_OK;
+}
+
+DMME_API int dmme_unet_plan_set_time_rows(dmme_plan* plan, const float* table, int64_t n_rows, float* cur_row) {
+    DMME_REQUIRE(plan, DMME_ERR_INVALID, "set_time_rows: null plan");
+    if (!cur_row) {
+        plan->trow_table = nullptr;
+        plan->trow_cur = nullptr;
+        plan->trow_n = 0;
+        return DMME_OK;
+    }
+    DMME_REQUIRE(table && n_rows > 0, DMME_ERR_INVALID, "set_time_rows: a current row without its table");
+    DMME_REQUIRE(!plan->cond && plan->cfg.arch != DMME_ARCH_CLASSIFIER, DMME_ERR_INVALID, "set_time_rows: a class-conditional plan or a classifier keeps its time path");
+    plan->trow_table = table;
+    plan->trow_cur = cur_row;
+    plan->trow_n = n_rows;
+    return DMME_OK;
+}
+
 static int unet_forward_impl(const dmme_plan* plan, const void* packed, const float* x, const int64_t* t, int t_len,
                       float* y, void* workspace, const float* drop_masks, void* stream, bool keep_ctx, const int64_t* labels = nullptr,
-                      int* status = nullptr) {
+                      int* status = nullptr, const float* trow = nullptr) {
     DMME_REQUIRE(plan && packed && x && t && y && workspace, DMME_ERR_INVALID, "unet_forward: null argument");
+    DMME_REQUIRE(!trow || (t_len == 1 && !keep_ctx && !plan->cond), DMME_ERR_INVALID, "unet_forward: time rows feed the no-grad walk of an unconditional plan at one timestep");
     DMME_REQUIRE((plan->cond != 0) == (labels != nullptr), DMME_ERR_INVALID,
                  plan->cond ? "unet_forward: a class-conditional plan (DMME_ARCH_DDPM_COND) takes labels: call dmme_unet_forward_cond / dmme_cfg_chain_step"
                             : "unet_forward_cond: the plan is not class-conditional (DMME_ARCH_DDPM_COND)");
@@ -1412,7 +1473,7 @@
         plan->nograd_ws = workspace;
     }
     for (int oi = 0; oi < (int)P->ops.size(); ++oi) {
-        const int rc = run_op(P, P->ops[oi], pk, x, t, P->cond && oi > P->label_op ? P->B : nt, y, ws, drop_masks, s, keep_ctx, labels, status);
+        const int rc = run_op(P, P->ops[oi], pk, x, t, P->cond && oi > P->label_op ? P->B : nt, y, ws, drop_masks, s, keep_ctx, labels, status, trow);
         if (rc != DMME_OK) return rc;
     }
     if (P->head_src >= 0) {
@@ -1529,6 +1590,13 @@
         if (numel_out) *numel_out = n;
         return DMME_OK;
     }
+    if (strcmp(name, "time_projection") == 0) {
+        const int64_t n = (int64_t)plan->B * plan->tproj_cols;
+        DMME_REQUIRE(n <= numel_cap, DMME_ERR_INVALID, "debug_read: destination too small");
+        DMME_CHECK_HIP(hipMemcpyAsync(dst, (const char*)workspace + plan->ws_tproj, (size_t)n * 4, hipMemcpyDeviceToDevice, s));
+        if (numel_out) *numel_out = n;
+        return DMME_OK;
+    }
     auto it = plan->named.find(name);
     DMME_REQUIRE(it != plan->named.end(), DMME_ERR_INVALID, "debug_read: unknown module '%s'", name);
     const Tensor& t = plan->tensors[it->second];
@@ -1624,6 +1692,14 @@
 DMME_API int dmme_chain_set(void* state, int64_t i, const int64_t* t_table, uint64_t philox_seed, uint64_t philox_offset, void* stream) {
     DMME_REQUIRE(state && t_table && i >= 0, DMME_ERR_INVALID, "chain_set: bad argument");
     return launch_chain_set(state, i, t_table, philox_seed, philox_offset, (hipStream_t)stream);
+}
+
+DMME_API int dmme_chain_set_rows(void* state, int64_t i, const int64_t* t_table, uint64_t philox_seed, uint64_t philox_offset, const float* table,
+                                 int64_t n_rows, int cols, float* cur_row, void* stream) {
+    DMME_REQUIRE(state && t_table && table && cur_row && cols > 0 && i < n_rows, DMME_ERR_INVALID, "chain_set_rows: bad argument (index %lld of %lld rows)",
+                 (long long)i, (long long)n_rows);
+    const ChainRows rows{table, cur_row, nullptr, cols};
+    return launch_chain_set(state, i, t_table, philox_seed, philox_offset, (hipStream_t)stream, &rows);
 }
 
 DMME_API int dmme_chain_update(int kind, float* x, const float* model_out, const float* step_coef, const int64_t* t_table, void* state,
@@ -1717,7 +1793,10 @@
     if (!cfg)
         if (int rc = lvl_check(plan, what, (hipStream_t)stream, true)) return rc;
     const int64_t* t_dev = (const int64_t*)state + 1;
-    if (int rc = unet_forward_impl(plan, packed, x, t_dev, 1, model_out, workspace, nullptr, stream, false, labels, status)) return rc;
+    const bool rows_on = plan->trow_cur && !plan->cond;
+    const ChainRows rows{plan->trow_table, plan->trow_cur, (unsigned*)((char*)workspace + plan->ws_mark), plan->tproj_cols};
+    if (int rc = unet_forward_impl(plan, packed, x, t_dev, 1, model_out, workspace, nullptr, stream, false, labels, status, rows_on ? plan->trow_cur : nullptr))
+        return rc;
     if (plan->pred != DMME_PRED_EPS)
         if (int rc = launch_pred_to_eps(plan->pred, model_out, x, plan->pred_ab, plan->pred_T, t_dev, 1, plan->B,
                                         (int64_t)plan->cfg.in_channels * plan->H * plan->W, (hipStream_t)stream))
@@ -1731,7 +1810,7 @@
         if (int rc = between()) return rc;
     return launch_sampler_chain(what, kind, sampler_operands(x, model_out, nullptr, cfg ? plan->B / 2 : plan->B, (int64_t)plan->cfg.in_channels * plan->H * plan->W,
                                                              grad, hist, planes, known, mask),
-                                step_coef, t_table, state, (hipStream_t)stream);
+                                step_coef, t_table, state, (hipStream_t)stream, rows_on ? &rows : nullptr);
 }
 
 DMME_API int dmme_chain_step(const dmme_plan* plan, const void* packed, float* x, float* model_out, void* workspace, int kind,
diff --git a/diffusion-models-made-easy_amd/csrc/plan_lvl.hip b/diffusion-models-made-easy_amd/csrc/plan_lvl.hip
--- a/diffusion-models-made-easy_amd/csrc/plan_lvl.hip
+++ b/diffusion-models-made-easy_amd/csrc/plan_lvl.hip
@@ -365,7 +365,8 @@
 static long long* g_lvl_stamps = nullptr;
 static int g_lvl_stamp_run = -1, g_lvl_stamp_wg = 0;
 
-int run_level(const dmme_plan* P, const LvlRun& R, const char* pk, char* ws, int nt, const float* drop_masks, hipStream_t s, bool keep_ctx) {
+int run_level(const dmme_plan* P, const LvlRun& R, const char* pk, char* ws, int nt, const float* drop_masks, hipStream_t s, bool keep_ctx,
+              const float* trow) {
     DMME_REQUIRE(R.ops_dev && R.sync_dev, DMME_ERR_INVALID, "level engine: the plan was created without a device");
     LvlArgs a{};
     a.ops = (!keep_ctx && R.ops_nograd_dev) ? R.ops_nograd_dev.get() : R.ops_dev.get();
@@ -373,7 +374,7 @@
     a.ws = ws;
     a.packed = pk;
     a.drop_masks = drop_masks;
-    a.tproj = (const float*)(ws + P->ws_tproj);
+    a.tproj = tproj_rows(P, ws, trow);
     a.tproj_ld = P->tproj_cols;
     a.nt = nt;
     a.N = P->B;
diff --git a/diffusion-models-made-easy_amd/diffusion_models/chain.py b/diffusion-models-made-easy_amd/diffusion_models/chain.py
--- a/diffusion-models-made-easy_amd/diffusion_models/chain.py
+++ b/diffusion-models-made-easy_amd/diffusion_models/chain.py
@@ -143,6 +143,41 @@
         self.graph = None
         self.capture_error = None
         self._wkey = None
+        lib = _lib.lib()
+        self.rows_n = int(self.ttab.numel())
+        self.rows_cols = int(lib.dmme_unet_plan_time_cols(self.plan.h))
+        nbytes = int(lib.dmme_unet_plan_time_rows_bytes(self.plan.h, self.rows_n))
+        self.rows_table = torch.empty(nbytes // 4, dtype=torch.float32, device=x.device) if nbytes else None
+        self.cur_row = torch.zeros(self.rows_cols, dtype=torch.float32, device=x.device) if nbytes else None
+        self._rows_key = None
+
+    def _time_rows(self, packed) -> bool:
+        if self.rows_table is None:
+            return False
+        key = (self.plan.packed_version, packed.data_ptr())
+        if self._rows_key == key:
+            return False
+        lib = _lib.lib()
+        scratch = torch.empty(int(lib.dmme_unet_time_rows_scratch_bytes(self.plan.h, self.rows_n)), dtype=torch.uint8, device=self.x.device)
+        _lib.check(lib.dmme_unet_time_rows(self.plan.h, _lib.ptr(packed), _lib.ptr(self.ttab), self.rows_n, _lib.ptr(self.rows_table), _lib.ptr(scratch),
+                                           _lib.stream_ptr()), "dmme_unet_time_rows")
+        self._rows_key = key
+        return True
+
+    def _set_rows(self, i: int, seed: int = 0, offset: int = 0):
+        _lib.check(_lib.lib().dmme_chain_set_rows(_lib.ptr(self.state), int(i), _lib.ptr(self.ttab), seed & 0xFFFFFFFFFFFFFFFF, int(offset), _lib.ptr(self.rows_table),
+                                                  self.rows_n, self.rows_cols, _lib.ptr(self.cur_row), _lib.stream_ptr()), "dmme_chain_set_rows")
+
+    def set(self, i: int, seed: int = 0, offset: int = 0):
+        if self.rows_table is None:
+            return super().set(i, seed, offset)
+        self._time_rows(self.model._packed_for(self.plan, fold=True))
+        self._set_rows(i, seed, offset)
+
+    def _set_time_rows(self, on: bool = True):
+        bound = on and self.rows_table is not None
+        _lib.check(_lib.lib().dmme_unet_plan_set_time_rows(self.plan.h, _lib.ptr(self.rows_table) if bound else None, self.rows_n if bound else 0,
+                                                           _lib.ptr(self.cur_row) if bound else None), "dmme_unet_plan_set_time_rows")
 
     def _set_prediction(self, plan=None):
         plan = self.plan if plan is None else plan
@@ -160,7 +195,11 @@
     def _launch(self, packed):
         self._set_prediction()
         self._set_threshold()
-        self._call(packed)
+        self._set_time_rows()
+        try:
+            self._call(packed)
+        finally:
+            self._set_time_rows(False)
         self.plan.overwritten()
 
     def _call(self, packed):
@@ -171,7 +210,7 @@
         )
 
     def _carried(self):
-        return [self.x, self.state]
+        return [self.x, self.state] + ([self.cur_row] if self.cur_row is not None else [])
 
     def _weights_key(self):
         return (self.plan.packed_version, self.plan.fold_version, self.plan.packed.data_ptr())
@@ -181,6 +220,8 @@
         if model.training:
             raise RuntimeError("ChainRunner: sampling chains run in eval mode (no dropout masks inside the replayed step)")
         packed = model._packed_for(self.plan, fold=True)
+        if self._time_rows(packed):
+            self._set_rows(-1)
         wkey = self._weights_key()
         if not self.use_graph or self.capture_error is not None:
             self._launch(packed)
diff --git a/include/dmme_hip.h b/include/dmme_hip.h
--- a/include/dmme_hip.h
+++ b/include/dmme_hip.h
@@ -193,6 +193,15 @@
 DMME_API int dmme_chain_update_gddim(float* x, const float* model_out, const float* noise, const float* step_coef, const int64_t* t_table,
                             void* state, int B, int64_t chw, void* stream);
 
+DMME_API int dmme_unet_plan_time_cols(const dmme_plan* plan);
+DMME_API int64_t dmme_unet_plan_time_rows_bytes(const dmme_plan* plan, int64_t n_rows);
+DMME_API int64_t dmme_unet_time_rows_scratch_bytes(const dmme_plan* plan, int64_t n_rows);
+DMME_API int dmme_unet_time_rows(const dmme_plan* plan, const void* packed, const int64_t* t_table, int64_t n_rows, float* table, void* scratch,
+                                 void* stream);
+DMME_API int dmme_unet_plan_set_time_rows(dmme_plan* plan, const float* table, int64_t n_rows, float* cur_row);
+DMME_API int dmme_chain_set_rows(void* state, int64_t i, const int64_t* t_table, uint64_t philox_seed, uint64_t philox_offset, const float* table,
+                                 int64_t n_rows, int cols, float* cur_row, void* stream);
+
 DMME_API int dmme_log_softmax_grad(const float* logits, const int64_t* y, int B, int K, int mode, float scale, float* loss, float* d_logits,
                                    int* status, void* stream);
 DMME_API int dmme_chain_update_guided(int kind, float* x, const float* model_out, const float* grad, const float* noise, const float* step_coef,
```

Result: no change. 476.0 denoising steps/s (one step = UNet forward + DDPM update on a batch of 128), summed over GPUs, median of 6 (+0.9%).
